# hahnyuan/PTQ4ViT

Measured on AMD Instinct MI355X. Metric: calibration throughput (wrapped modules calibrated per second), ViT-B/224 W8A8, 32 calibration images, higher is better.
Workload: dtype int8

## Files before the change

### include/ptq4vit_hip_debug.h

```cpp
#ifndef PTQ4VIT_HIP_DEBUG_H
#define PTQ4VIT_HIP_DEBUG_H

#include <stddef.h>
#include <stdint.h>

#ifdef __cplusplus
extern "C" {
#endif

int p4v_debug_set_variant(int variant, int force_generic);
int p4v_debug_set_tuning(int key, int value);
int p4v_debug_bound_totals(float* out, int64_t capacity, int64_t* count);
int p4v_debug_set_arena_gap(size_t bytes);
int p4v_debug_arena_ranges(uint64_t* out, int cap);
int p4v_debug_sos_sweep(const p4v_matmul_desc* desc, const float* d_A, const float* d_B, const float* d_out, const float* d_grad,
                        int n_cands, int c_lo, int c_hi, int known_cands, float* d_scores, void* d_workspace, size_t workspace_bytes,
                        void* stream);
int p4v_debug_topk_rows(const float* d_mass, int segs, int n, int k, int32_t* d_idx, void* stream);
int p4v_debug_pack_dual(const float* d_x, long rows, long cols, long cols_padded, int sos, int lo, int hi, int qmax,
                        const float* d_scale, float const_scale, int8_t* d_q1, int8_t* d_q2, void* stream);
int p4v_debug_pack_cands(const float* d_x, long rows, long cols, long rows_padded, long cols_padded, int layout, int lo, int hi,
                         const float* d_scales, int n_cands, const int* d_crange, const unsigned char* d_done, int live_max,
                         int general, int8_t* d_q, void* stream);
int p4v_debug_gather_im2col(int batch, int in_channels, int height, int width, int kernel_h, int kernel_w, int stride_h, int stride_w,
                            int pad_h, int pad_w, int dil_h, int dil_w, const float* d_x, const int32_t* d_idx, int k, float* d_dst,
                            void* stream);
int p4v_debug_prep_epi6(const float* d_o, const float* d_wt, const float* d_bias, long o_ss, long o_ts, int sr, int tr,
                        int bias_on_t, int wt_mode, int transposed, float* d_e, void* stream);

#ifdef __cplusplus
}
#endif
#endif
```

### ptq4vit_amd/_lib.py

```python
import ctypes as C
import os

_HERE = os.path.dirname(os.path.abspath(__file__))
LIB_PATH = os.environ.get("P4V_LIB") or os.path.join(_HERE, "csrc", "libptq4vit_hip.so")

METRICS = {
    "L1_norm": 0,
    "L2_norm": 1,
    "linear_weighted_L2_norm": 2,
    "square_weighted_L2_norm": 3,
    "hessian": 4,
    "cosine": 5,
}


class LinearDesc(C.Structure):
    _fields_ = [(n, C.c_int32) for n in (
        "batch", "tokens", "in_features", "out_features", "n_V", "n_H", "n_a", "w_bit", "a_bit", "metric",
        "eq_n", "search_round", "twin_postgelu", "init_layerwise", "has_bias", "reserved")]


class MatMulDesc(C.Structure):
    _fields_ = ([(n, C.c_int32) for n in ("batch", "heads", "M", "K", "N")] + [("_pad0", C.c_int32)] +
                [("a_stride", C.c_int64 * 4), ("b_stride", C.c_int64 * 4)] +
                [(n, C.c_int32) for n in ("A_bit", "B_bit", "metric", "eq_n", "search_round", "sos",
                                          "init_layerwise", "reserved")])


class MatMulBlocksDesc(C.Structure):
    _fields_ = [("mm", MatMulDesc)] + [(n, C.c_int32) for n in ("n_V_A", "n_H_A", "n_V_B", "n_H_B")]


class ConvDesc(C.Structure):
    _fields_ = [(n, C.c_int32) for n in (
        "batch", "in_channels", "height", "width", "out_channels", "kernel_h", "kernel_w", "stride_h", "stride_w",
        "pad_h", "pad_w", "dil_h", "dil_w", "w_bit", "a_bit", "metric", "eq_n", "search_round", "channelwise",
        "init_layerwise", "has_bias", "reserved")]


class KernelStats(C.Structure):
    _fields_ = [("sweep_i8_ms", C.c_double), ("sweep_i8_launches", C.c_int64), ("sweep_i8_macs", C.c_double),
                ("sweep_f32_ms", C.c_double), ("sweep_f32_launches", C.c_int64), ("sweep_f32_macs", C.c_double),
                ("sweep_i8_alg_macs", C.c_double), ("sweep_f32_alg_macs", C.c_double),
                ("sweep6_ms", C.c_double), ("sweep6_launches", C.c_int64), ("sweep6_macs", C.c_double), ("sweep6_alg_macs", C.c_double),
                ("memo_hits", C.c_int64), ("memo_misses", C.c_int64),
                ("sweep7_ms", C.c_double), ("sweep7_launches", C.c_int64), ("sweep7_macs", C.c_double), ("sweep7_alg_macs", C.c_double),
                ("sweep7_twin_ms", C.c_double), ("sweep7_twin_launches", C.c_int64), ("event_overhead_ms", C.c_double)]


class LaunchRecord(C.Structure):
    _fields_ = [("kind", C.c_int32), ("stage", C.c_int32), ("grid_x", C.c_int32), ("grid_z", C.c_int32),
                ("ms", C.c_double), ("ops", C.c_double), ("alg_ops", C.c_double), ("alg_bytes", C.c_double)]


LAUNCH_KINDS = {0: "k_sweep<int8>", 1: "k_sweep<float>", 2: "k_sweep6", 3: "k_sweep7", 4: "k_sweep7 (twin)", 5: "k_sweep4/5", 6: "k_sweep9",
                7: "k_sweep8", 8: "k_sweep2g", 9: "k_sweep2", 11: "k_sos_split", 12: "k_bound", 13: "k_slice_b", 14: "k_slice_a", 15: "k_sweep_seg"}
LAUNCH_STAGES = {0: "full", 1: "A", 2: "B1", 3: "B2", 4: "A2"}


class PlaneDesc(C.Structure):
    _fields_ = [("rows", C.c_int64), ("cols", C.c_int64), ("cols_padded", C.c_int64), ("rows_per_scale", C.c_int64),
                ("mode", C.c_int32), ("lo", C.c_int32), ("hi", C.c_int32), ("qmax", C.c_int32),
                ("const_scale", C.c_float), ("reserved", C.c_int32)]


class ExportDesc(C.Structure):
    _fields_ = [("dims", C.c_int32 * 4), ("src_stride", C.c_int64 * 4),
                ("scale1_stride", C.c_int64 * 4), ("scale1_div", C.c_int32 * 4),
                ("scale2_stride", C.c_int64 * 4), ("scale2_div", C.c_int32 * 4),
                ("scale2_const", C.c_float),
                ("mode", C.c_int32), ("lo1", C.c_int32), ("hi1", C.c_int32), ("lo2", C.c_int32), ("hi2", C.c_int32),
                ("qmax", C.c_int32), ("reserved", C.c_int32)]


class GroupJob(C.Structure):
    _fields_ = [("kind", C.c_int32), ("status", C.c_int32), ("desc", C.c_void_p), ("inp", C.c_void_p * 5), ("mult", C.c_void_p),
                ("out", C.c_void_p * 3), ("workspace", C.c_void_p), ("workspace_bytes", C.c_size_t)]


JOB_LINEAR, JOB_MATMUL, JOB_CONV, JOB_MATMUL_BLOCKS = 0, 1, 2, 3
PLANE_SYM, PLANE_SOS_HI, PLANE_SOS_LO, PLANE_TWIN = 1, 2, 3, 4
EXPORT_SYM_I8, EXPORT_SYM_F32, EXPORT_GELU_U8, EXPORT_SOS_U8 = 0, 1, 2, 3


EXPORTS = [
    "p4v_version", "p4v_last_error",
    "p4v_linear_workspace_bytes", "p4v_linear_calibrate",
    "p4v_matmul_workspace_bytes", "p4v_matmul_calibrate",
    "p4v_matmul_blocks_workspace_bytes", "p4v_matmul_blocks_calibrate", "p4v_amax_init_matmul_blocks",
    "p4v_matmul_blocks_search", "p4v_matmul_blocks_quant_forward",
    "p4v_conv_workspace_bytes", "p4v_conv_calibrate",
    "p4v_calibrate_group", "p4v_launch_counters",
    "p4v_linear_quant_forward", "p4v_matmul_quant_forward",
    "p4v_amax_init_linear", "p4v_linear_search_w", "p4v_linear_search_a",
    "p4v_amax_init_matmul", "p4v_matmul_search_A", "p4v_sos_search_split", "p4v_matmul_search_B",
    "p4v_amax_init_conv", "p4v_conv_search_w_channelwise", "p4v_conv_search_w_layerwise", "p4v_conv_search_a",
    "p4v_score_argmax_gather",
    "p4v_quantize_i8", "p4v_pack_plane_i8", "p4v_fake_quant", "p4v_export_quantize", "p4v_multi_copy",
    "p4v_stats_enable", "p4v_stats_reset", "p4v_stats_get", "p4v_stats_launches", "p4v_prune_counters",
    "p4v_debug_set_variant", "p4v_debug_set_tuning", "p4v_debug_bound_totals", "p4v_debug_topk_rows", "p4v_debug_pack_dual", "p4v_debug_prep_epi6",
    "p4v_debug_pack_cands", "p4v_debug_gather_im2col", "p4v_debug_sos_sweep",
    "p4v_debug_set_arena_gap", "p4v_debug_arena_ranges",
]

_lib = None


def load():
    global _lib
    if _lib is not None:
        return _lib
    if not os.path.exists(LIB_PATH):
        raise RuntimeError(
            f"ptq4vit_amd: HIP extension {LIB_PATH} is missing -- build it with "
            "`python -c 'import __graft_entry__ as g; g.build()'` (hipcc --offload-arch=gfx950). "
            "There is no CPU fallback for the calibration path.")
    import torch
    lib = C.CDLL(LIB_PATH)
    vp, fp, ip = C.c_void_p, C.c_void_p, C.c_void_p
    lib.p4v_version.restype = C.c_int
    lib.p4v_last_error.restype = C.c_char_p
    lib.p4v_linear_workspace_bytes.restype = C.c_size_t
    lib.p4v_linear_workspace_bytes.argtypes = [C.POINTER(LinearDesc)]
    lib.p4v_linear_calibrate.restype = C.c_int
    lib.p4v_linear_calibrate.argtypes = [C.POINTER(LinearDesc), fp, fp, fp, fp, fp, fp, fp, fp, fp, ip, vp, C.c_size_t, vp]
    lib.p4v_matmul_workspace_bytes.restype = C.c_size_t
    lib.p4v_matmul_workspace_bytes.argtypes = [C.POINTER(MatMulDesc)]
    lib.p4v_matmul_calibrate.restype = C.c_int
    lib.p4v_matmul_calibrate.argtypes = [C.POINTER(MatMulDesc), fp, fp, fp, fp, fp, fp, fp, fp, fp, ip, vp, C.c_size_t, vp]
    MBD = C.POINTER(MatMulBlocksDesc)
    lib.p4v_matmul_blocks_workspace_bytes.restype = C.c_size_t
    lib.p4v_matmul_blocks_workspace_bytes.argtypes = [MBD]
    lib.p4v_matmul_blocks_calibrate.restype = C.c_int
    lib.p4v_matmul_blocks_calibrate.argtypes = [MBD, fp, fp, fp, fp, fp, fp, fp, fp, fp, ip, vp, C.c_size_t, vp]
    lib.p4v_amax_init_matmul_blocks.restype = C.c_int
    lib.p4v_amax_init_matmul_blocks.argtypes = [MBD, fp, fp, fp, fp, vp, C.c_size_t, vp]
    lib.p4v_matmul_blocks_search.restype = C.c_int
    lib.p4v_matmul_blocks_search.argtypes = [MBD, C.c_int32, C.c_int32, C.c_int32] + [fp] * 9 + [ip, vp, C.c_size_t, vp]
    lib.p4v_matmul_blocks_quant_forward.restype = C.c_int
    lib.p4v_matmul_blocks_quant_forward.argtypes = [MBD, fp, fp, fp, fp, fp, fp, vp, C.c_size_t, vp]
    lib.p4v_conv_workspace_bytes.restype = C.c_size_t
    lib.p4v_conv_workspace_bytes.argtypes = [C.POINTER(ConvDesc)]
    lib.p4v_conv_calibrate.restype = C.c_int
    lib.p4v_conv_calibrate.argtypes = [C.POINTER(ConvDesc), fp, fp, fp, fp, fp, fp, fp, fp, fp, ip, vp, C.c_size_t, vp]
    lib.p4v_linear_quant_forward.restype = C.c_int
    lib.p4v_linear_quant_forward.argtypes = [C.POINTER(LinearDesc), fp, fp, fp, fp, fp, fp, vp, C.c_size_t, vp]
    lib.p4v_matmul_quant_forward.restype = C.c_int
    lib.p4v_matmul_quant_forward.argtypes = [C.POINTER(MatMulDesc), fp, fp, fp, fp, fp, fp, vp, C.c_size_t, vp]
    LD, MD, CD = C.POINTER(LinearDesc), C.POINTER(MatMulDesc), C.POINTER(ConvDesc)
    tail = [vp, C.c_size_t, vp]
    for name, args in (
            ("p4v_amax_init_linear", [LD] + [fp] * 4),
            ("p4v_linear_search_w", [LD] + [fp] * 9 + [ip]),
            ("p4v_linear_search_a", [LD] + [fp] * 9 + [ip]),
            ("p4v_amax_init_matmul", [MD] + [fp] * 4),
            ("p4v_matmul_search_A", [MD] + [fp] * 8 + [ip]),
            ("p4v_sos_search_split", [MD] + [fp] * 7 + [ip]),
            ("p4v_matmul_search_B", [MD] + [fp] * 9 + [ip]),
            ("p4v_amax_init_conv", [CD] + [fp] * 4),
            ("p4v_conv_search_w_channelwise", [CD] + [fp] * 9 + [ip]),
            ("p4v_conv_search_w_layerwise", [CD] + [fp] * 9 + [ip]),
            ("p4v_conv_search_a", [CD] + [fp] * 9 + [ip])):
        fn = getattr(lib, name)
        fn.restype = C.c_int
        fn.argtypes = args + tail
    lib.p4v_score_argmax_gather.restype = C.c_int
    lib.p4v_score_argmax_gather.argtypes = [fp, C.c_int32, C.c_int32, fp, fp, ip, vp]
    lib.p4v_quantize_i8.restype = C.c_int
    lib.p4v_quantize_i8.argtypes = [fp, C.c_int64, C.c_int64, C.c_int64, fp, C.c_int64, C.c_int32, C.c_int32, vp, vp]
    lib.p4v_fake_quant.restype = C.c_int
    lib.p4v_fake_quant.argtypes = [fp, C.c_int64, C.c_int64, fp, C.c_int64, C.c_int32, C.c_int32, fp, vp]
    lib.p4v_pack_plane_i8.restype = C.c_int
    lib.p4v_pack_plane_i8.argtypes = [C.POINTER(PlaneDesc), fp, fp, vp, vp]
    lib.p4v_export_quantize.restype = C.c_int
    lib.p4v_export_quantize.argtypes = [C.POINTER(ExportDesc), fp, fp, fp, vp, vp]
    lib.p4v_multi_copy.restype = C.c_int
    lib.p4v_multi_copy.argtypes = [vp, C.c_int32, C.c_int64, C.c_int64, vp]
    lib.p4v_debug_topk_rows.restype = C.c_int
    lib.p4v_debug_topk_rows.argtypes = [vp, C.c_int, C.c_int, C.c_int, vp, vp]
    lib.p4v_debug_pack_dual.restype = C.c_int
    lib.p4v_debug_pack_dual.argtypes = [fp, C.c_long, C.c_long, C.c_long, C.c_int, C.c_int, C.c_int, C.c_int, fp, C.c_float, vp, vp, vp]
    lib.p4v_debug_pack_cands.restype = C.c_int
    lib.p4v_debug_pack_cands.argtypes = [fp, C.c_long, C.c_long, C.c_long, C.c_long, C.c_int, C.c_int, C.c_int, fp, C.c_int, vp, vp,
                                         C.c_int, C.c_int, vp, vp]
    lib.p4v_debug_gather_im2col.restype = C.c_int
    lib.p4v_debug_gather_im2col.argtypes = [C.c_int] * 12 + [fp, ip, C.c_int, fp, vp]
    lib.p4v_debug_sos_sweep.restype = C.c_int
    lib.p4v_debug_sos_sweep.argtypes = [C.POINTER(MatMulDesc), fp, fp, fp, fp, C.c_int, C.c_int, C.c_int, C.c_int, fp, vp, C.c_size_t, vp]
    lib.p4v_debug_prep_epi6.restype = C.c_int
    lib.p4v_debug_prep_epi6.argtypes = [fp, fp, fp, C.c_long, C.c_long, C.c_int, C.c_int, C.c_int, C.c_int, C.c_int, fp, vp]
    lib.p4v_debug_set_variant.restype = C.c_int
    lib.p4v_debug_set_variant.argtypes = [C.c_int, C.c_int]
    lib.p4v_debug_set_tuning.restype = C.c_int
    lib.p4v_debug_set_tuning.argtypes = [C.c_int, C.c_int]
    lib.p4v_debug_set_arena_gap.restype = C.c_int
    lib.p4v_debug_set_arena_gap.argtypes = [C.c_size_t]
    lib.p4v_debug_arena_ranges.restype = C.c_int
    lib.p4v_debug_arena_ranges.argtypes = [C.POINTER(C.c_uint64), C.c_int]
    lib.p4v_debug_bound_totals.restype = C.c_int
    lib.p4v_debug_bound_totals.argtypes = [fp, C.c_int64, C.POINTER(C.c_int64)]
    lib.p4v_stats_enable.restype = C.c_int
    lib.p4v_stats_enable.argtypes = [C.c_int]
    lib.p4v_stats_reset.restype = C.c_int
    lib.p4v_stats_get.restype = C.c_int
    lib.p4v_stats_get.argtypes = [C.POINTER(KernelStats)]
    lib.p4v_stats_launches.restype = C.c_int
    lib.p4v_stats_launches.argtypes = [C.POINTER(LaunchRecord), C.c_int64, C.POINTER(C.c_int64)]
    lib.p4v_prune_counters.restype = C.c_int
    lib.p4v_prune_counters.argtypes = [C.POINTER(C.c_int64), C.c_int]
    lib.p4v_launch_counters.restype = C.c_int
    lib.p4v_launch_counters.argtypes = [C.POINTER(C.c_int64), C.c_int]
    lib.p4v_calibrate_group.restype = C.c_int
    lib.p4v_calibrate_group.argtypes = [C.POINTER(GroupJob), C.c_int32, vp, vp]
    _lib = lib
    return lib


def check(rc, what):
    if rc != 0:
        msg = load().p4v_last_error().decode("utf-8", "replace")
        if rc == -2:
            raise NotImplementedError(f"{what}: {msg}")
        raise RuntimeError(f"{what} failed (code {rc}): {msg}")


def source_hash():
    import hashlib
    root = os.path.dirname(os.path.abspath(__file__))
    h = hashlib.sha256()
    for rel in ("csrc/p4v_kernels.h", "csrc/p4v_api.hip", "../include/ptq4vit_hip.h"):
        with open(os.path.join(root, rel), "rb") as f:
            h.update(f.read())
    return h.hexdigest()[:16]
```

### ptq4vit_amd/csrc/p4v_api.hip

```cpp
#include <hip/hip_runtime.h>

#include <algorithm>
#include <atomic>
#include <climits>
#include <cstdarg>
#include <cstdio>
#include <condition_variable>
#include <cstring>
#include <deque>
#include <functional>
#include <thread>
#include <mutex>
#include <string>
#include <unordered_map>
#include <type_traits>
#include <vector>

#include "../../include/ptq4vit_hip.h"
#include "../../include/ptq4vit_hip_debug.h"
#include "p4v_kernels.h"

using namespace p4v;

namespace {
// ... 4 lines not shown
    char buf[512];
    va_list ap;
    va_start(ap, fmt);
    vsnprintf(buf, sizeof buf, fmt, ap);
    va_end(ap);
    g_err = buf;
    return code;
}

#define HIPCHK(expr)                                                                              \
    do {                                                                                          \
        hipError_t e_ = (expr);                                                                   \
        if (e_ != hipSuccess) return fail(P4V_ERR_HIP, "%s failed: %s", #expr, hipGetErrorString(e_)); \
    } while (0)
#define CHK(expr)              \
    do {                       \
        int r_ = (expr);       \
        if (r_ != 0) return r_; \
    } while (0)

inline long rup(long x, long m) { return (x + m - 1) / m * m; }
inline int cdiv(long a, long b) { return (int)((a + b - 1) / b); }

constexpr size_t WS_ALIGN = 16;
std::atomic<size_t> g_arena_gap{0};
thread_local std::vector<std::pair<size_t, size_t>> g_arena_ranges;
inline void arena_note(size_t b, size_t e) {
    if (e <= b) return;
    auto& v = g_arena_ranges;
    auto it = v.begin();
    while (it != v.end() && it->second < b) ++it;
    if (it == v.end() || it->first > e) { v.insert(it, {b, e}); return; }
    it->first = std::min(it->first, b);
    it->second = std::max(it->second, e);
    auto nx = it + 1;
    while (nx != v.end() && nx->first <= it->second) { it->second = std::max(it->second, nx->second); nx = v.erase(nx); }
}

struct Arena {
    char* base;
    size_t cap, off, peak;
    size_t top;
    bool dry;
    size_t gap;
    Arena(void* b, size_t c) : base((char*)b), cap(c & ~(size_t)255), off(0), peak(0), top(0), dry(b == nullptr),
                               gap(g_arena_gap.load(std::memory_order_relaxed)) {
        if (!dry) g_arena_ranges.clear();
    }
    template <typename T> T* get(size_t n) {
        off = (size_t)rup((long)off, 256);
        T* p = dry ? nullptr : (T*)(base + off);
        if (gap && !dry) arena_note(off, off + n * sizeof(T));
        off += n * sizeof(T) + gap;
        if (off + top > peak) peak = off + top;
        return p;
    }
    char* get_top(size_t bytes) {
        top += (size_t)rup((long)bytes, 256) + gap;
        if (off + top > peak) peak = off + top;
        if (dry || top > cap) return nullptr;
        if (gap) arena_note(cap - top, cap - top + bytes);
        return base + cap - top;
    }
    bool ok() const { return dry || off + top <= cap; }
};

struct StatRec { hipEvent_t a, b; int kind; double macs, alg; int stage, gx, gz; double ms, bytes; };
thread_local double g_alg_bytes = 0;
thread_local double g_alg_macs_cand = 0;
thread_local double g_exec_frac = 1.0;
thread_local bool g_stat_on = false;
thread_local std::vector<StatRec> g_stat_recs;
thread_local std::vector<StatRec> g_stat_done;
thread_local bool g_b1_keep = false;
thread_local std::vector<float> g_b1_totals;
thread_local int g_stage = 0;
thread_local p4v_kernel_stats g_stats = {};
thread_local long g_memo_hits = 0, g_memo_misses = 0;
std::atomic<long long> g_prune_cnt[4];
constexpr int VARIANT_KEPT = 1 | 2 | 4 | 2048 | 32768 | 65536 | 131072 | 524288 | 1048576 | 2097152 | 4194304 | 8388608 | 134217728;
std::atomic<int> g_variant_word{0};
#define g_variant (g_variant_word.load(std::memory_order_relaxed) & 0x3fffffff)
#define g_force_v1 ((g_variant_word.load(std::memory_order_relaxed) >> 30) & 1)
std::atomic<int> g_tune[16];
enum { TUNE_CG6 = 0, TUNE_CG2 = 1, TUNE_CG2G = 2, TUNE_CG7 = 3, TUNE_PRINT = 4, TUNE_ORDER7 = 5, TUNE_P6 = 6, TUNE_PLANE_GIB = 7, TUNE_EPI6W = 8,
       TUNE_LOOSE_PCT = 9, TUNE_SLICE_DIV = 10, TUNE_SLICE_SMALL = 11, TUNE_B1_PATH = 12, TUNE_TIER2 = 13, TUNE_TIER2_DIV = 14, TUNE_LOOSE_ROWS = 15 };
inline bool tune_b1_removed(int v) { return v == 1 || v == 2 || v == 3 || v == 5 || v == 6 || v == 8 || v == 10 || v == 12; }
inline int tune(int k) { return g_tune[k].load(std::memory_order_relaxed); }
inline bool b1_previous() { return tune(TUNE_B1_PATH) == 4; }

inline int ws_aligned(const void* p) {
    return ((uintptr_t)p % WS_ALIGN) == 0 ? 0 : fail(P4V_ERR_INVALID, "d_workspace must be aligned to %zu bytes", WS_ALIGN);
}

struct Group;
struct Ctx {
    hipStream_t st;
    Arena ws;
    bool dry;
    Group* grp = nullptr;
    int slot = 0;
    int par = 1;
};

struct StatInfo { int kind; double macs, alg; int stage, gx, gz; double bytes; };
struct QOp;
struct KernelDesc {
    hipError_t (*one)(const QOp&, hipStream_t);
    hipError_t (*many)(const QOp* const*, int, hipStream_t);
    int cap;
};
constexpr int QOP_PARAM_BYTES = 480;
struct QOp {
    enum Type : int { KERNEL, FILL, D2H, H2D, COPY2D, WAIT };
    int type = KERNEL;
    const KernelDesc* kd = nullptr;
    dim3 grid, block;
    unsigned lds = 0;
    alignas(16) char params[QOP_PARAM_BYTES];
    void* dst = nullptr; const void* src = nullptr; size_t bytes = 0; int value = 0;
    size_t dpitch = 0, spitch = 0, width = 0, height = 0;
    std::vector<char> payload;
    bool timed = false;
    bool heavy = false;
    StatInfo si{};
};
inline hipError_t lds_attr(const void* fn, unsigned lds, std::atomic<bool>& done) {
    if (lds <= 48 * 1024 || done.load(std::memory_order_acquire)) return hipSuccess;
    const hipError_t e = hipFuncSetAttribute(fn, hipFuncAttributeMaxDynamicSharedMemorySize, 160 * 1024);
    if (e == hipSuccess) done.store(true, std::memory_order_release);
    return e;
}
template <typename P, void (*K1)(P), void (*KG)(GroupArgs<P>)> struct Kern {
    static_assert(sizeof(P) <= QOP_PARAM_BYTES, "kernel parameter block larger than a queued operation holds");
    static hipError_t one(const QOp& op, hipStream_t st) {
        static std::atomic<bool> attr{false};
        if (hipError_t e = lds_attr((const void*)K1, op.lds, attr); e != hipSuccess) return e;
        P p;
        std::memcpy(&p, op.params, sizeof(P));
        void* args[] = {&p};
        return hipLaunchKernel((const void*)K1, op.grid, op.block, args, op.lds, st);
    }
    static hipError_t many(const QOp* const* ops, int n, hipStream_t st) {
        static std::atomic<bool> attr{false};
        GroupArgs<P> a;
        unsigned off = 0, lds = 0;
        a.n = n;
        for (int m = 0; m < n; ++m) {
            const QOp& op = *ops[m];
            a.off[m] = off; a.gx[m] = op.grid.x; a.gy[m] = op.grid.y; a.gz[m] = op.grid.z;
            std::memcpy(&a.p[m], op.params, sizeof(P));
            off += (unsigned)rup((long)op.grid.x * op.grid.y * op.grid.z, 8);
            lds = std::max(lds, op.lds);
        }
        a.off[n] = off;
        if (hipError_t e = lds_attr((const void*)KG, lds, attr); e != hipSuccess) return e;
        void* args[] = {&a};
        return hipLaunchKernel((const void*)KG, dim3(off), ops[0]->block, args, lds, st);
    }
    static const KernelDesc* desc() { static const KernelDesc d{&one, &many, GroupArgs<P>::CAP}; return &d; }
};
template <typename P, void (*K1)(P)> struct Kern1 {
    static_assert(sizeof(P) <= QOP_PARAM_BYTES, "kernel parameter block larger than a queued operation holds");
    static hipError_t one(const QOp& op, hipStream_t st) {
        static std::atomic<bool> attr{false};
        if (hipError_t e = lds_attr((const void*)K1, op.lds, attr); e != hipSuccess) return e;
        P p;
        std::memcpy(&p, op.params, sizeof(P));
        void* args[] = {&p};
        return hipLaunchKernel((const void*)K1, op.grid, op.block, args, op.lds, st);
    }
    static const KernelDesc* desc() { static const KernelDesc d{&one, nullptr, 1}; return &d; }
};
#define KERN(P, NAME) (Kern<P, NAME, NAME##_g>::desc())
#define KERN_T(P, NAME, ...) (Kern<P, NAME<__VA_ARGS__>, NAME##_g<__VA_ARGS__>>::desc())
#define KERN1_T(P, NAME, ...) (Kern1<P, NAME<__VA_ARGS__>>::desc())

constexpr int MIR_SLOT = 2048, MIR_SLOTS = 3;
constexpr int MIR_HDR = 160, MIR_BLK = 32, MIR_RB1 = 16, MIR_RB2 = 80;
constexpr size_t MIRROR_BYTES = sizeof(int) * MIR_HDR + sizeof(float) * MIR_SLOT * MIR_SLOTS;
inline int* mirror_alloc() {
    void* p = nullptr;
    if (hipHostMalloc(&p, MIRROR_BYTES, hipHostMallocPortable | hipHostMallocMapped | hipHostMallocCoherent) != hipSuccess) { (void)hipGetLastError(); p = nullptr; }
    return (int*)p;
}

struct Group {
    hipStream_t st = nullptr;
    int n = 0;
    std::mutex mu;
    std::condition_variable cv;
    std::vector<std::deque<QOp>> q;
    std::vector<int> state;
    int blocked = 0;
    unsigned long gen = 0;
    int status = 0;
    std::string err;
    std::vector<int*> mirrors;
    bool stat_on = false;
    std::vector<StatRec>* stat_recs = nullptr;
    long n_ops = 0, n_launches = 0, n_rounds = 0;
    hipEvent_t inputs_ready = nullptr;
    bool waited = false;
    int last_par[16] = {};
    int issue_kernels(std::vector<const QOp*>& ops);
    int issue_round();
    int sync(int slot);
    void finish(int slot);
};

std::atomic<long long> g_launch_cnt[4];
int enqueue_now(hipStream_t st, const QOp& op, bool timed, std::vector<StatRec>* recs) {
    g_launch_cnt[1].fetch_add(1, std::memory_order_relaxed);
    StatRec rec{};
    if (timed) {
        HIPCHK(hipEventCreate(&rec.a));
        HIPCHK(hipEventCreate(&rec.b));
        HIPCHK(hipEventRecord(rec.a, st));
    }
    HIPCHK(op.kd->one(op, st));
    if (timed) {
        HIPCHK(hipEventRecord(rec.b, st));
        rec.kind = op.si.kind; rec.macs = op.si.macs; rec.alg = op.si.alg; rec.stage = op.si.stage; rec.gx = op.si.gx; rec.gz = op.si.gz; rec.bytes = op.si.bytes;
        recs->push_back(rec);
    }
    return 0;
}
int issue_plain(hipStream_t st, const QOp& op) {
    switch (op.type) {
        case QOp::FILL: HIPCHK(hipMemsetAsync(op.dst, op.value, op.bytes, st)); break;
        case QOp::D2H: HIPCHK(hipMemcpyAsync(op.dst, op.src, op.bytes, hipMemcpyDeviceToHost, st)); break;
        case QOp::H2D: HIPCHK(hipMemcpyAsync(op.dst, op.payload.data(), op.bytes, hipMemcpyHostToDevice, st)); break;
        case QOp::COPY2D: HIPCHK(hipMemcpy2DAsync(op.dst, op.dpitch, op.src, op.spitch, op.width, op.height, hipMemcpyDeviceToDevice, st)); break;
        default: break;
    }
    return 0;
}
int Group::issue_kernels(std::vector<const QOp*>& ops) {
    const KernelDesc* kd = ops[0]->kd;
    const int total = (int)ops.size();
    if (ops[0]->heavy && ops[0]->si.kind >= 0 && ops[0]->si.kind < 16) last_par[ops[0]->si.kind] = total;
    if (!kd->many || total == 1) {
        for (const QOp* op : ops) { CHK(enqueue_now(st, *op, op->timed && stat_recs, stat_recs)); ++n_launches; }
        return 0;
    }
    const int chunks = cdiv(total, kd->cap), per = cdiv(total, chunks);
    for (int i0 = 0; i0 < total; i0 += per) {
        const int m = std::min(per, total - i0);
        bool timed = stat_recs != nullptr;
        for (int i = 0; i < m; ++i) timed = timed && ops[i0 + i]->timed;
        StatRec rec{};
        if (timed) {
            HIPCHK(hipEventCreate(&rec.a));
            HIPCHK(hipEventCreate(&rec.b));
            HIPCHK(hipEventRecord(rec.a, st));
        }
        HIPCHK(kd->many(ops.data() + i0, m, st));
        g_launch_cnt[1].fetch_add(1, std::memory_order_relaxed);
        ++n_launches;
        if (timed) {
            HIPCHK(hipEventRecord(rec.b, st));
            const StatInfo& s0 = ops[i0]->si;
            rec.kind = s0.kind; rec.stage = s0.stage; rec.gz = m;
            for (int i = 0; i < m; ++i) {
                const QOp& o = *ops[i0 + i];
                rec.macs += o.si.macs; rec.alg += o.si.alg; rec.bytes += o.si.bytes;
                rec.gx += (int)rup((long)o.grid.x * o.grid.y * o.grid.z, 8);
            }
            stat_recs->push_back(rec);
        }
    }
    return 0;
}
int Group::issue_round() {
    ++n_rounds;
    g_launch_cnt[2].fetch_add(1, std::memory_order_relaxed);
    std::vector<const QOp*> bucket;
    for (;;) {
        int best = -1, best_n = 0;
        bool best_heavy = true;
        int n_wait = 0, n_live = 0;
        for (int i = 0; i < n; ++i) {
            if (q[i].empty()) continue;
            ++n_live;
            const QOp& h = q[i].front();
            if (h.type == QOp::WAIT) { ++n_wait; continue; }
            if (h.type != QOp::KERNEL) { best = i; best_n = 0; break; }
            if (h.heavy && !best_heavy) continue;
            int cnt = 0;
            for (int j = i; j < n; ++j)
                if (!q[j].empty()) { const QOp& o = q[j].front(); cnt += o.type == QOp::KERNEL && o.kd == h.kd && o.block.x == h.block.x && o.block.y == h.block.y && o.block.z == h.block.z; }
            if ((best_heavy && !h.heavy) || cnt > best_n) { best = i; best_n = cnt; best_heavy = h.heavy; }
        }
        if (best < 0 && n_wait > 0) {
            if (!waited && inputs_ready) { HIPCHK(hipStreamWaitEvent(st, inputs_ready, 0)); waited = true; }
            for (int i = 0; i < n; ++i)
                if (!q[i].empty() && q[i].front().type == QOp::WAIT) q[i].pop_front();
            continue;
        }
        if (best < 0) break;
        const QOp& h = q[best].front();
        if (h.type != QOp::KERNEL) {
            const int r = issue_plain(st, h);
            ++n_ops;
            q[best].pop_front();
            if (r) return r;
            continue;
        }
        bucket.clear();
        std::vector<int> who;
        for (int j = best; j < n; ++j)
            if (!q[j].empty()) { const QOp& o = q[j].front(); if (o.type == QOp::KERNEL && o.kd == h.kd && o.block.x == h.block.x && o.block.y == h.block.y && o.block.z == h.block.z) { bucket.push_back(&o); who.push_back(j); } }
        n_ops += (long)bucket.size();
        const int r = issue_kernels(bucket);
        for (int j : who) q[j].pop_front();
        if (r) return r;
    }
    return 0;
}
int Group::sync(int slot) {
    std::unique_lock<std::mutex> lk(mu);
    state[slot] = 1;
    ++blocked;
    if (blocked == n) {
// ... 114 lines not shown
        case P4V_METRIC_LINEAR_WEIGHTED_L2: *epi = EPI_W_SQ; *wt_mode = 3; break;
        case P4V_METRIC_SQUARE_WEIGHTED_L2: *epi = EPI_SQ_W; *wt_mode = 2; break;
        case P4V_METRIC_HESSIAN: *epi = EPI_SQ_W; *wt_mode = 1; break;
        default: *epi = EPI_COS; *wt_mode = 0; break;
    }
}

int launch_absmax(Ctx& c, const float* src, const long (&st)[4], int D0, int D1, int R, int C, int nV, int nH,
                  int crb_r, int crb_c, int signed_max, unsigned* out) {
    if (c.dry) return 0;
    CHK(q_fill(c, out, 0, sizeof(unsigned) * (size_t)D1 * nV * nH));
    AbsMaxParams p{src, st[0], st[1], st[2], st[3], D0, D1, R, C, nV, nH, crb_r, crb_c, 0, signed_max, out};
    p.row_tile = std::max(1, std::min(crb_r, std::max(1, 8192 / std::max(1, std::min(crb_c, C)))));
    const int tiles_per_v = cdiv(crb_r, p.row_tile);
    dim3 grid(tiles_per_v * nV * nH, D1, D0);
    return enqueue(c, KERN(AbsMaxParams, k_absmax), grid, dim3(256), 0, p);
}

int launch_interval(Ctx& c, const unsigned* enc, int n, float denom, int broadcast, float* interval) {
    if (c.dry) return 0;
    return enqueue(c, KERN(IntervalParams, k_interval_from_max), dim3(cdiv(n, 64)), dim3(64), 0, IntervalParams{enc, n, denom, broadcast, interval});
}

int launch_cands(Ctx& c, const float* mult, const float* interval, int ncand, int nblk, float* cands) {
    if (c.dry) return 0;
    return enqueue(c, KERN(CandsParams, k_make_cands), dim3(cdiv((long)ncand * nblk, 256)), dim3(256), 0, CandsParams{mult, interval, ncand, nblk, cands});
}

int launch_scale(Ctx& c, ScaleParams p) {
    if (c.dry) return 0;
    return enqueue(c, KERN(ScaleParams, k_scale_table), dim3(cdiv((long)p.C * p.nblk, 256)), dim3(256), 0, p);
}

std::atomic<int> g_cvt_state{0};
void cvt_probe(hipStream_t stream) {
    if (g_cvt_state.load(std::memory_order_acquire) != 0) return;
    static std::mutex mu;
    std::lock_guard<std::mutex> lk(mu);
    if (g_cvt_state.load(std::memory_order_acquire) != 0) return;
    static unsigned* scratch = nullptr;
    if (!scratch && hipMalloc(&scratch, 8 * sizeof(unsigned)) != hipSuccess) { (void)hipGetLastError(); scratch = nullptr; return; }
    unsigned h[5] = {9, 9, 9, 9, 9};
    hipLaunchKernelGGL(k_probe_cvt, dim3(1), dim3(64), 0, stream, scratch);
    if (hipGetLastError() != hipSuccess || hipMemcpyAsync(h, scratch, sizeof h, hipMemcpyDeviceToHost, stream) != hipSuccess ||
        hipStreamSynchronize(stream) != hipSuccess) { (void)hipGetLastError(); return; }
    const bool sat = h[3] == 0 && h[4] == 255;
    const int st = (sat && h[0] == 0 && h[1] == 1 && h[2] == 2) ? 1 : (sat && h[0] == 1 && h[1] == 2 && (h[2] == 2 || h[2] == 3)) ? 2 : 3;
    if (tune(TUNE_PRINT) > 0) fprintf(stderr, "[p4v] v_cvt_pk_u8_f32(0.7, 1.5, 2.5, -3, 300) = %u %u %u %u %u -> mode %d\n", h[0], h[1], h[2], h[3], h[4], st);
    g_cvt_state.store(st, std::memory_order_release);
}
float cvt_bias(Ctx& c) {
    if (!c.dry && !c.grp) cvt_probe(c.st);
    const int st = g_cvt_state.load(std::memory_order_acquire);
    return st == 1 ? 128.5f : st == 2 ? 128.0f : 0.0f;
}
inline bool pack1_ok(const PackParams& p, int live_max) {
    return p.mode == PACK_SYM && !p.conv && !(p.blk_mode == 1 && p.blk_div2) && p.lo >= -128 && p.hi <= 127 && p.lo <= p.hi &&
           (p.crange ? live_max == 1 : p.C == 1) && (p.c_inner != 3 || (p.Rp % 64 == 0 && p.Kp % 64 == 0));
}
std::atomic<int> g_pack_general{0};
template <typename T> int launch_pack(Ctx& c, const PackParams& p_, int live_max = -1) {
    if (c.dry) return 0;
    PackParams p = p_;
    if (p.crange && live_max == 0) return 0;
    p.qbias = (sizeof(T) == 1 && p.mode == PACK_SYM && p.lo == -128 && p.hi == 127 && tune(TUNE_B1_PATH) != 11) ? cvt_bias(c) : 0.0f;
    const long total = (long)p.Z * p.Rp * (p.Kp / 16);
    if (total >= (1L << 31)) return fail(P4V_ERR_UNSUPPORTED, "operand plane too large for k_pack (%ld 16-element runs)", total);
    const int groups = cdiv((p.crange && live_max > 0) ? std::min(p.C, live_max) : p.C, PACK_CG);
    const long cap = !p.crange ? 256L * 64 : live_max > 0 ? std::max(256L * 12, 256L * 64 / groups) : 256L * 12;
    const int blocks = (int)std::min<long>(cdiv(total, 256), cap);
    if (p.mode == PACK_TWIN_I8) {
        if (sizeof(T) != 1 || p.C != 1 || p.c_inner != 0 || !p.scales || p.conv || p.zdiv > 0)
            return fail(P4V_ERR_UNSUPPORTED, "merged twin plane: one fixed row-major int8 plane only");
        return enqueue(c, KERN(PackParams, k_pack_twin), dim3(blocks), dim3(256), 0, p);
    }
    const bool single = sizeof(T) == 1 && pack1_ok(p, live_max) && !g_pack_general.load(std::memory_order_relaxed);
    if (tune(TUNE_PRINT) > 1) fprintf(stderr, "[p4v] %s stage %d: Z %d Rp %d Kp %d C %d crange %d done %d live_max %d layout %d grid %d x %d\n", single ? "k_pack1" : "k_pack", g_stage, p.Z, p.Rp, p.Kp, p.C, p.crange != nullptr, p.done != nullptr, live_max, p.c_inner, blocks, single ? 1 : groups);
    if (single) return enqueue(c, KERN(PackParams, k_pack1), dim3(blocks), dim3(256), 0, p);
    return enqueue(c, KERN_T(PackParams, k_pack, T), dim3(blocks, groups), dim3(256), 0, p);
}

inline int lockstep(const Ctx& c, int kind) {
    if (!c.grp) return 1;
    const int seen = (kind >= 0 && kind < 16) ? c.grp->last_par[kind] : 0;
    return std::max(1, seen > 0 ? seen : c.par);
}
inline int cu_slots(const Ctx& c, int slots, int kind) { return std::max(8, slots / lockstep(c, kind)); }
#define P4V_EPI4(epi, X)                                   \
    switch (epi) {                                         \
        case EPI_SQ_W: { constexpr int E = EPI_SQ_W; X; }  \
        case EPI_SQ: { constexpr int E = EPI_SQ; X; }      \
        case EPI_ABS: { constexpr int E = EPI_ABS; X; }    \
        default: { constexpr int E = EPI_W_SQ; X; }        \
    }

template <typename T, bool TWIN> int launch_sweep_epi(Ctx& c, const SweepParams& p, int epi, int cgroups, const StatInfo* si) {
    const size_t lds = 2 * (TWIN ? 3 : 2) * SW_TILE_BYTES;
    dim3 grid(p.mtiles * p.ntiles, p.Z, cgroups), block(512);
    switch (epi) {
        case EPI_SQ_W: return enqueue(c, KERN_T(SweepParams, k_sweep, T, TWIN, EPI_SQ_W), grid, block, lds, p, si);
        case EPI_SQ: return enqueue(c, KERN_T(SweepParams, k_sweep, T, TWIN, EPI_SQ), grid, block, lds, p, si);
        case EPI_ABS: return enqueue(c, KERN_T(SweepParams, k_sweep, T, TWIN, EPI_ABS), grid, block, lds, p, si);
        case EPI_W_SQ: return enqueue(c, KERN_T(SweepParams, k_sweep, T, TWIN, EPI_W_SQ), grid, block, lds, p, si);
        case EPI_STORE: return enqueue(c, KERN1_T(SweepParams, k_sweep, T, TWIN, EPI_STORE), grid, block, lds, p, si);
        case EPI_FWD: return enqueue(c, KERN1_T(SweepParams, k_sweep, T, TWIN, EPI_FWD), grid, block, lds, p, si);
        default: return enqueue(c, KERN1_T(SweepParams, k_sweep, T, TWIN, EPI_COS), grid, block, lds, p, si);
    }
}

template <bool TWIN> int launch_sweep2g_epi(Ctx& c, const SweepParams& p, int epi, int cgroups, const StatInfo* si) {
    const int per = 2 * cdiv(p.c1 - p.c0, 2 * cgroups);
    const size_t lds = (size_t)SW2_NS * (TWIN ? 4 : 3) * SW2_TILE + (size_t)per * 8 * sizeof(float) * (TWIN ? 3 : 2);
    dim3 grid(p.mtiles * p.ntiles, p.Z, cgroups), block(512);
    P4V_EPI4(epi, return enqueue(c, KERN_T(SweepParams, k_sweep2g, TWIN, E), grid, block, lds, p, si))
}

template <bool TWIN> int launch_sweep2_epi(Ctx& c, const SweepParams& p, int epi, int cgroups, const StatInfo* si) {
    const int per = cdiv(p.c1 - p.c0, cgroups);
    const size_t lds = (size_t)SW2_NS * (TWIN ? 3 : 2) * SW2_TILE + (size_t)per * 8 * sizeof(float) * (TWIN ? 3 : 2);
    dim3 grid(p.mtiles * p.ntiles, p.Z, cgroups), block(512);
    switch (epi) {
        case EPI_SQ_W: return enqueue(c, KERN_T(SweepParams, k_sweep2, TWIN, EPI_SQ_W), grid, block, lds, p, si);
        case EPI_SQ: return enqueue(c, KERN_T(SweepParams, k_sweep2, TWIN, EPI_SQ), grid, block, lds, p, si);
        case EPI_ABS: return enqueue(c, KERN_T(SweepParams, k_sweep2, TWIN, EPI_ABS), grid, block, lds, p, si);
        case EPI_FWD: return enqueue(c, KERN1_T(SweepParams, k_sweep2, TWIN, EPI_FWD), grid, block, lds, p, si);
        case EPI_STORE:
            if constexpr (TWIN) return enqueue(c, KERN1_T(SweepParams, k_sweep2, TWIN, EPI_STORE), grid, block, lds, p, si);
            else return enqueue(c, KERN_T(SweepParams, k_sweep2, TWIN, EPI_STORE), grid, block, lds, p, si);
        case EPI_COS: return enqueue(c, KERN_T(SweepParams, k_sweep2, TWIN, EPI_COS), grid, block, lds, p, si);
        default: return enqueue(c, KERN_T(SweepParams, k_sweep2, TWIN, EPI_W_SQ), grid, block, lds, p, si);
    }
}

#ifdef P4V_TRACE
unsigned long long* g_trace = nullptr;
int trace_attach(Sweep3Params& p) {
    if (!g_trace) HIPCHK(hipMalloc(&g_trace, sizeof(unsigned long long) * 16 * 65536));
    p.trace = g_trace;
    return 0;
}
int trace_dump(Ctx& c, dim3 grid, int ktiles) {
    if (!getenv("P4V_TRACE_FILE")) return 0;
    const size_t n = (size_t)grid.x * grid.z * 16;
    HIPCHK(hipStreamSynchronize(c.st));
    std::vector<unsigned long long> h(n);
    HIPCHK(hipMemcpy(h.data(), g_trace, n * 8, hipMemcpyDeviceToHost));
    FILE* f = fopen(getenv("P4V_TRACE_FILE"), "ab");
    unsigned long long hdr[4] = {0xABCDull, grid.x, grid.z, (unsigned long long)ktiles};
    fwrite(hdr, 8, 4, f); fwrite(h.data(), 8, n, f); fclose(f);
    return 0;
}
#endif

inline StatInfo stat_info(int kind, double macs, double alg, int gx, int gz, double bytes) {
    return StatInfo{kind, macs * g_exec_frac, alg * g_exec_frac, g_stage, gx, gz, bytes};
}

enum SweepKind { SK_BOUND, SK_SWEEP6, SK_SWEEP5, SK_SWEEP7, SK_SWEEP7_TWIN, SK_SWEEP7_MERGED, SK_SWEEP9, SK_SWEEP8, SK_SWEEP2G, SK_SWEEP2,
                 SK_GENERIC_I8, SK_GENERIC_F32, SK_COUNT };
constexpr int SWEEP_RECORD_KIND[SK_COUNT] = {12, 2, 5, 3, 4, 4, 6, 7, 8, 9, 0, 1};
inline bool sweep_stationary(SweepKind k) { return k == SK_SWEEP6 || k == SK_SWEEP5; }
inline bool sweep_large_k(SweepKind k) { return k == SK_SWEEP7 || k == SK_SWEEP7_TWIN || k == SK_SWEEP7_MERGED; }

int launch_sweep5(Ctx& c, const Sweep3Params& p, int epi, int cgroups) {
    if (c.dry) return 0;
    const int per = 2 * cdiv(p.c1 - p.c0, 2 * cgroups);
    const size_t lds = (size_t)p.ktiles * SW2_TILE + (size_t)SW5_NP * 2 * SW2_TILE + (size_t)per * 8 * sizeof(float) * 2 + 256;
// ... 176 lines not shown
}

struct PlaneCache {
    char* buf = nullptr;
    bool assigned = false, valid = false;
    unsigned char* done = nullptr;
};
struct SliceCache {
    bool assigned = false;
    int k = 0;
    int k_eff = 0;
    int* idx = nullptr; float* mass = nullptr; float* mass_u = nullptr;
    float* Os = nullptr; float* Gs = nullptr; float* Rs = nullptr; float* Cs = nullptr;
    const void* idx_src = nullptr; int idx_wt = -1;
    const void* o_src = nullptr; const void* g_src = nullptr; const void* r_src = nullptr; const void* c_src = nullptr;
    float* frac = nullptr;
    PlaneCache aplane;
    bool loose = false;
    float frac_host = 1.0f;
};
typedef PlaneCache EpiCache;

struct Operand {
    PackParams pk;
    bool expanded;
    bool present;
};

struct SegPlan {
    SegTable seg; unsigned char ablk[SEG_MAX], bblk[SEG_MAX]; int Kseg;
    int batch, H, M, K, N;
    int nVA, nHA, nVB, nHB, crA, ccA, crB, ccB;
    const float* A; long a_st[4]; const float* B; long b_st[4];
    int Aq, Bq; bool sos;
    const float* ivA; const float* ivB;
    const float* split;
    int side, ov_v, ov_h;
    const float* cands; int cand_cs, cand_hs;
    bool b_shared;
};

struct Pass {
    bool i8, twin;
    int epi, wt_mode;
    Operand row, row2, col;
    int Z;
    long row_zs_shared, col_zs_shared;
    int Mrows, Ncols, K;
    int eq_n;
    ScaleParams s1, s2;
    bool use_s1;
    int sb_mode, sb_div, s_cs;
    const float* bias; int bias_axis; long bias_zs;
    const float* O; const float* G;
    long o_zs, o_bs, o_ms, o_nbs, o_ns; int o_inner, o_ninner;
    int j_mode, j_div, nj; double norm;
    int cos_ZB, cos_ZV, cos_j_mode, cos_j_div;
    const float* cands; int cand_cs, cand_js, cand_off;
    float* interval; int out_js, out_off;
    float* aux_out; float aux_div;
    float* scores_out; int scores_out_ld;
    int32_t* best_out;
    float* store_out;
    bool cos6;
    bool cos7;
    bool twin_disjoint;
    const int* crange;
    const int* crange_blk;
    int host_lo, host_hi;
    const int* host_rblk;
    int host_len;
    float* scores_keep;
    bool no_select;
    bool prunable;
    bool prunable_f32;
    float* S1_pre; float* S2_pre; bool s_ready;
    SliceCache* scache;
    SliceCache* scache2;
    bool bound_kernel;
    bool host_sync_ok;
    PlaneCache* cache;
    EpiCache* ecache;
    bool pack_only;
    const SegPlan* seg;
};

static const long PLANE_BUDGET_DEFAULT = 6L << 30;
#define PLANE_BUDGET (tune(TUNE_PLANE_GIB) > 0 ? ((long)tune(TUNE_PLANE_GIB) << 30) : PLANE_BUDGET_DEFAULT)
#define PLANE_CACHE_MAX (PLANE_BUDGET / 2)

int choose_cgroups(long wgs, int ncand, int ktiles, int slots, double prologue_us, double tile_us, int cg_max = 25) {
    int best = 1;
    double best_t = 1e30;
    for (int cg = 1; cg <= std::min(ncand, cg_max); ++cg) {
        const long rounds = (wgs * cg + slots - 1) / slots;
        const double t = (double)rounds * (prologue_us + (double)cdiv(ncand, cg) * ktiles * tile_us);
        if (t < best_t * 0.999) { best_t = t; best = cg; }
    }
    return best;
}

bool dual_pack_ok(const PackParams& a, const PackParams& b) {
    auto plain = [](const PackParams& p) {
        return (p.mode == PACK_SYM || p.mode == PACK_SOS_HI || p.mode == PACK_SOS_LO) && p.blk_mode == 0 && !p.conv && !p.crange;
    };
    return plain(a) && plain(b) && a.src == b.src && a.R == b.R && a.K == b.K && a.s_r == b.s_r && a.s_k == b.s_k &&
           a.s_z == b.s_z && a.s_z2 == b.s_z2 && a.zdiv == b.zdiv;
}

int launch_pass_select(Ctx& c, const Pass& ps, const float* scores) {
    SelectParams sl{scores, ps.eq_n, ps.nj, ps.cands, ps.cand_cs, ps.cand_js, ps.cand_off, ps.interval, ps.out_js,
                    ps.out_off, ps.aux_out, ps.aux_div, ps.scores_out, ps.scores_out_ld, ps.best_out};
    return launch_select(c, sl);
}

int launch_pack_seg(Ctx& c, PackSegParams p) {
    if (c.dry) return 0;
    p.qbias = (p.mode == PACK_SYM && p.lo == -128 && p.hi == 127) ? cvt_bias(c) : 0.0f;
    const long total = (long)p.Z * p.Rp * (p.Kseg / 16);
    if (total >= (1L << 31)) return fail(P4V_ERR_UNSUPPORTED, "operand plane too large for k_pack_seg (%ld 16-element runs)", total);
    const int groups = cdiv(p.C, PACK_CG);
    return enqueue(c, KERN(PackSegParams, k_pack_seg), dim3((unsigned)std::min<long>(cdiv(total, 256), 256L * 64), groups), dim3(256), 0, p);
}
template <bool TWIN> int launch_sweep_seg_epi(Ctx& c, const SweepSegParams& p, int epi, int cgroups, const StatInfo* si) {
    const size_t lds = 2 * (TWIN ? 3 : 2) * SW_TILE_BYTES + 2 * SEG_MAX * 128 * sizeof(float) + SEG_KT_MAX * sizeof(short) + 2 * SEG_MAX;
    dim3 grid(p.mtiles * p.ntiles, p.Z, cgroups), block(512);
    if (epi == EPI_FWD) return enqueue(c, KERN_T(SweepSegParams, k_sweep_seg, TWIN, EPI_FWD), grid, block, lds, p, si);
    if constexpr (!TWIN) { if (epi == EPI_COS) return enqueue(c, KERN_T(SweepSegParams, k_sweep_seg, false, EPI_COS), grid, block, lds, p, si); }
    if (epi == EPI_COS) return fail(P4V_ERR_UNSUPPORTED, "k_sweep_seg: the cosine epilogue has no twin instance");
    P4V_EPI4(epi, return enqueue(c, KERN_T(SweepSegParams, k_sweep_seg, TWIN, E), grid, block, lds, p, si))
}
int run_pass_seg(Ctx& c, Pass& ps) {
    const SegPlan& g = *ps.seg;
    const int Z = ps.Z, M = g.M, N = g.N, H = g.H, Kseg = g.Kseg;
    const bool fwd = ps.epi == EPI_FWD, cosm = ps.epi == EPI_COS;
    const int ZB = g.b_shared ? 1 : Z;
    g_alg_macs_cand = (double)M * N * g.K * Z;
    g_alg_bytes = 4.0 * ((double)M * g.K * Z + (double)N * g.K * ZB) + (ps.G ? 8.0 : 4.0) * (double)M * N * Z;
    const int Mp = (int)rup(M, SW_BM), Np = (int)rup(N, SW_BN), MT = cosm ? cdiv(M, 64) : Mp / 64;
    const long a_plane = (long)Z * Mp * Kseg, b_plane = (long)ZB * Np * Kseg;
    const bool a_exp = g.side == 1, b_exp = g.side == 2;
    const long exp_plane = a_exp ? a_plane : b_plane;
    const int chunk = (int)std::max<long>(1, std::min<long>(ps.eq_n, PLANE_BUDGET / std::max<long>(1, exp_plane)));
    const size_t mark = c.ws.off;
    char* abuf = c.ws.get<char>((size_t)a_plane * (a_exp ? chunk : 1));
    char* a2buf = g.sos ? c.ws.get<char>((size_t)a_plane) : nullptr;
    char* bbuf = c.ws.get<char>((size_t)b_plane * (b_exp ? chunk : 1));
    const long p_zs = (long)MT * Np * (cosm ? 3 : 1), p_cs = p_zs * Z;
    float* part = fwd ? nullptr : c.ws.get<float>((size_t)p_cs * ps.eq_n);
    float* scores = fwd ? nullptr : c.ws.get<float>((size_t)ps.eq_n * H);
    if (!c.ws.ok()) return fail(P4V_ERR_WORKSPACE, "workspace too small: need >= %zu bytes", c.ws.off);
    if (c.dry) { c.ws.off = mark; return 0; }

    auto a_pack = [&](int mode, char* dst, const float* cands, int C) {
        PackSegParams p{};
        p.src = g.A; p.s_z2 = g.a_st[0]; p.s_z = g.a_st[1]; p.s_r = g.a_st[2]; p.s_k = g.a_st[3]; p.zdiv = H;
        p.Z = Z; p.R = M; p.K = g.K; p.Rp = Mp; p.Kseg = Kseg; p.dst = dst; p.C = C;
        p.H = H; p.mode = mode; p.seg = g.seg;
        std::memcpy(p.kblk, g.ablk, sizeof p.kblk);
        if (mode == PACK_SYM) {
            p.iv = g.ivA; p.iv_hs = g.nVA * g.nHA; p.iv_rs = g.nHA; p.iv_ks = 1; p.r_div = g.crA; p.nblk_r = g.nVA;
            p.cands = cands; p.cand_cs = g.cand_cs; p.cand_hs = g.cand_hs; p.ov_r = g.ov_v; p.ov_k = g.ov_h;
            p.lo = -g.Aq; p.hi = g.Aq - 1;
        } else {
            p.iv = g.split; p.iv_hs = p.iv_rs = p.iv_ks = 0; p.r_div = std::max(1, M); p.nblk_r = 1;
            p.qm1 = (float)(g.Aq - 1);
// ... 391 lines not shown
    return launch_sweep7(c, q, pl.kind == SK_SWEEP7_MERGED ? 2 : ps.twin ? 1 : 0, ps.epi, cg7);
}

int sweep_chunk_tiled(Ctx& c, const Pass& ps, const SweepPlan& pl, const PassBufs& b, SweepKind kind, int c0, int nc) {
    const int esz = pl.esz, Mp = pl.Mp, Np = pl.Np, Kp = pl.Kp;
    SweepParams sp{};
    sp.a_cs = ps.row.expanded ? pl.row_plane1 : 0;
    sp.A = b.row - (long)c0 * sp.a_cs;
    sp.a_zs = ps.row_zs_shared ? 0 : (long)Mp * Kp * esz;
    if (ps.twin) {
        sp.a2_cs = ps.row2.expanded ? pl.row_plane1 : 0;
        sp.A2 = b.row2 - (long)c0 * sp.a2_cs;
        sp.a2_zs = sp.a_zs;
    }
    sp.b_cs = ps.col.expanded ? pl.col_plane1 : 0;
    sp.B = b.col - (long)c0 * sp.b_cs;
    sp.b_zs = ps.col_zs_shared ? 0 : (long)pl.NpB * Kp * esz;
    sp.b_rows = pl.b64 ? 64 : 0;
    sp.ldk = Kp * esz; sp.ktiles = sp.ldk / SW_BKB;
    sp.S1 = b.S1; sp.S2 = b.S2; sp.s_cs = ps.s_cs; sp.sb_mode = ps.sb_mode; sp.sb_div = std::max(1, ps.sb_div);
    sp.bias = ps.bias; sp.bias_axis = ps.bias_axis; sp.bias_zs = ps.bias_zs;
    sp.O = ps.O; sp.Wt = ps.G ? ps.G : ps.O; sp.wt_mode = ps.wt_mode;
    sp.o_zs = ps.o_zs; sp.o_bs = ps.o_bs; sp.o_ms = ps.o_ms; sp.o_nbs = ps.o_nbs; sp.o_ns = ps.o_ns;
    sp.o_inner = ps.o_inner > 0 ? ps.o_inner : INT_MAX;
    sp.o_ninner = ps.o_ninner > 0 ? ps.o_ninner : INT_MAX;
    sp.M = ps.Mrows; sp.N = ps.Ncols; sp.Z = ps.Z; sp.c0 = c0; sp.c1 = c0 + nc; sp.crange = ps.crange;
    sp.crange_blk = pl.rblk_z; sp.cb_div = std::max(1, ps.j_div);
    sp.part = b.part; sp.p_cs = pl.p_cs; sp.p_zs = pl.p_zs; sp.Np = pl.NpP;
    sp.mtiles = Mp / SW_BM; sp.ntiles = Np / SW_BN;
    sp.dbg = g_variant & 3;
    sp.store = ps.store_out;
    const long wgs = (long)sp.mtiles * sp.ntiles * ps.Z;
    int cgroups;
    switch (kind) {
        case SK_GENERIC_I8: case SK_GENERIC_F32:
            cgroups = choose_cgroups(wgs, nc, sp.ktiles, cu_slots(c, 512, SWEEP_RECORD_KIND[kind]), 20.0, ps.i8 ? 1.6 : 2.6);
            break;
        case SK_SWEEP9:
            sp.halves = pl.h9;
            sp.rows_p_stream = sp.a_cs == 0 ? Np : Mp;
            cgroups = choose_cgroups((long)pl.h9 * ps.Z, nc, 1, cu_slots(c, SW9_NW == 4 ? 512 : 256, SWEEP_RECORD_KIND[SK_SWEEP9]), 12.0, 0.9);
            break;
        case SK_BOUND:
            sp.bound = 1;
            sp.dbg = tune(TUNE_B1_PATH) >= 16 ? (tune(TUNE_B1_PATH) >> 4) : 0;
            sp.A = b.row; sp.B = b.col; sp.a_cs = sp.b_cs = 0;
            [[fallthrough]];
        default:
            cgroups = choose_cgroups(wgs, nc, sp.ktiles, cu_slots(c, ps.twin ? 256 : 512, SWEEP_RECORD_KIND[SK_SWEEP2]), ps.twin ? 40.0 : 25.0, ps.twin ? 0.45 : 0.40);
    }
    const bool tuned = kind != SK_GENERIC_I8 && kind != SK_GENERIC_F32 && !pl.fast_cos && !ps.store_out;
    if (tuned) {
        const char* g = kind == SK_SWEEP2G ? "g" : "";
        if (const int t_ = tune(kind == SK_SWEEP2G ? TUNE_CG2G : TUNE_CG2); t_ > 0) cgroups = std::max(1, std::min(nc, t_));
        if (tune(TUNE_PRINT) > 0) fprintf(stderr, "[p4v] sweep2%s tiles %d x %d z %d ktiles %d cand %d twin %d -> cgroups %d\n", g, sp.mtiles, sp.ntiles, ps.Z, sp.ktiles, nc, (int)ps.twin, cgroups);
    }
    return launch_sweep(c, sp, kind, ps.twin, ps.epi, cgroups);
}

int finish_pass(Ctx& c, const Pass& ps, const SweepPlan& pl, const PassBufs& b) {
    if (ps.epi == EPI_COS) {
        FinishCosParams fp{b.part, pl.p_cs, pl.fin_zs, pl.fin_ld, pl.fin_rows, ps.cos_ZB, ps.cos_ZV, pl.fin_cols, ps.eq_n,
                           ps.cos_j_mode, pl.fin_jdiv, ps.nj, ps.norm, b.scores};
        return launch_finish_cos(c, fp);
    }
    FinishParams fp{b.part, pl.p_cs, pl.fin_zs, pl.fin_ld, pl.fin_rows, ps.Z, pl.fin_cols, ps.eq_n, ps.j_mode, pl.fin_jdiv, ps.nj, ps.norm,
                    b.scores, ps.crange};
    if (ps.crange && b.pc && b.pc->done) { fp.mark_done = b.pc->done; fp.mark_n = ps.eq_n; }
    fp.crange_blk = pl.rblk ? pl.rblk : pl.rblk_z;
    return launch_finish(c, fp);
}

int run_pass(Ctx& c, Pass& ps) {
    if (ps.seg) return run_pass_seg(c, ps);
    g_alg_macs_cand = (double)ps.Mrows * ps.Ncols * ps.K * ps.Z;
    g_alg_bytes = 4.0 * ((double)ps.Mrows * ps.K * (ps.row_zs_shared ? 1 : ps.Z) + (double)ps.Ncols * ps.K * (ps.col_zs_shared ? 1 : ps.Z)) +
                  (ps.G ? 8.0 : 4.0) * (double)ps.Mrows * ps.Ncols * ps.Z;
    SweepPlan pl;
    CHK(plan_sweep(c, ps, pl));
    const size_t mark = c.ws.off;
    PassBufs b{};
    CHK(pass_workspace(c, ps, pl, b));
    if (ps.pack_only) {
        if (b.pc && ps.row.expanded != ps.col.expanded && !ps.crange) CHK(pack_expanded(c, ps, pl, b, 0, ps.eq_n));
        c.ws.off = mark;
        return 0;
    }
    CHK(prep_epilogue(c, ps, pl, b));
    if (ps.use_s1 && !ps.s_ready) {
        ps.s1.S = b.S1; ps.s1.C = ps.eq_n; ps.s1.nblk = ps.s_cs;
        CHK(launch_scale(c, ps.s1));
        if (ps.twin) { ps.s2.S = b.S2; ps.s2.C = ps.eq_n; ps.s2.nblk = ps.s_cs; CHK(launch_scale(c, ps.s2)); }
    }
    CHK(pack_fixed_planes(c, ps, pl, b));
    for (int c0 = 0; c0 < ps.eq_n; c0 += pl.chunk) {
        const int nc = std::min(pl.chunk, ps.eq_n - c0);
        CHK(pack_expanded(c, ps, pl, b, c0, nc));
        CHK(chunk_exec_frac(c, ps, pl, c0, nc));
        const SweepKind kind = chunk_kind(pl, nc);
        if (sweep_stationary(kind)) CHK(sweep_chunk_stationary(c, ps, pl, b, c0, nc));
        else if (sweep_large_k(kind)) CHK(sweep_chunk_large_k(c, ps, pl, b, c0, nc));
        else CHK(sweep_chunk_tiled(c, ps, pl, b, kind, c0, nc));
    }
    g_exec_frac = 1.0;
    if (!ps.store_out) {
        CHK(finish_pass(c, ps, pl, b));
        if (!ps.no_select) CHK(launch_pass_select(c, ps, b.scores));
    }
    c.ws.off = mark;
    return 0;
}

struct SliceGeo {
    bool lin; int segs, seg_rows, k , Ncols, K;
    const float* O; const float* G; int wt_mode; long o_ms;
    const float* row_src; long s_r, s_k; int zdiv; long s_z2, s_z;
    bool conv; PackParams conv_pk;
    int k_cap;
};
int slice_alloc(Ctx& c, SliceCache* sc, const SliceGeo& g, bool keep, bool bump) {
    if (sc->assigned) {
        if (sc->k != g.k_cap) return fail(P4V_ERR_INVALID, "slice cache reused with another geometry");
        return 0;
    }
    if (!keep && !bump) return 0;
    const long zrows = (long)g.segs * g.seg_rows, out_elems = (long)g.segs * g.k_cap * g.Ncols, row_elems = (long)g.segs * g.k_cap * g.K;
    if (keep) {
        sc->idx = reinterpret_cast<int*>(c.ws.get_top((size_t)g.segs * g.k_cap * sizeof(int)));
        sc->mass = reinterpret_cast<float*>(c.ws.get_top((size_t)zrows * sizeof(float)));
        sc->Os = reinterpret_cast<float*>(c.ws.get_top((size_t)out_elems * sizeof(float)));
        sc->Gs = reinterpret_cast<float*>(c.ws.get_top((size_t)out_elems * sizeof(float)));
        sc->Rs = reinterpret_cast<float*>(c.ws.get_top((size_t)row_elems * sizeof(float)));
        sc->frac = reinterpret_cast<float*>(c.ws.get_top(256));
        sc->assigned = true;
    } else {
        sc->idx = c.ws.get<int>((size_t)g.segs * g.k_cap);
        sc->mass = c.ws.get<float>((size_t)zrows);
        sc->Os = c.ws.get<float>((size_t)out_elems);
        sc->Gs = c.ws.get<float>((size_t)out_elems);
        sc->Rs = c.ws.get<float>((size_t)row_elems);
    }
    sc->k = g.k_cap;
    return 0;
}
int slice_fill(Ctx& c, SliceCache* sc, const SliceGeo& g, bool host_sync_ok) {
    const long zrows = (long)g.segs * g.seg_rows;
    const void* wsrc = g.G ? (const void*)g.G : (const void*)g.O;
    const bool new_idx = sc->idx_src != wsrc || sc->idx_wt != g.wt_mode || (g.wt_mode != 1 && sc->o_src != g.O);
    if (new_idx) {
        CHK(enqueue(c, KERN(RowMassParams, k_row_mass), dim3((unsigned)cdiv(zrows, 4)), dim3(256), 0, RowMassParams{g.G ? g.G : g.O, g.O, zrows, (long)g.Ncols, g.wt_mode, sc->mass}));
        CHK(enqueue(c, KERN(TopkParams, k_topk_rows), dim3(g.segs), dim3(1024), 0, TopkParams{sc->mass, g.seg_rows, g.k, sc->idx}));
        sc->idx_src = wsrc; sc->idx_wt = g.wt_mode;
        sc->o_src = sc->g_src = sc->r_src = nullptr;
        if (sc->frac && host_sync_ok && !(g_variant & 8388608)) {
            float f = 1.0f;
            int* hm = host_mirror(c);
            CHK(enqueue(c, KERN(MassFracParams, k_mass_fraction), dim3(1), dim3(1024), 0,
                        MassFracParams{sc->mass, zrows, sc->idx, g.segs, g.seg_rows, g.k, sc->frac, hm ? reinterpret_cast<float*>(hm + 4) : nullptr}));
            if (!hm) CHK(q_d2h(c, &f, sc->frac, sizeof f));
            CHK(q_sync(c));
            if (hm) f = *reinterpret_cast<volatile float*>(hm + 4);
            if (tune(TUNE_PRINT) > 0) fprintf(stderr, "[p4v] slice holds %.4f of the metric weight (%d x %d of %d rows)\n", f, g.segs, g.k, g.seg_rows);
            sc->frac_host = f;
            if (g.k < g.k_cap && !(f >= 0.97f)) {
                SliceGeo g2 = g;
                g2.k = g.k_cap;
                sc->idx_src = nullptr;
// ... 79 lines not shown
        pk.Rp = 16; pk.Kp = Kp; pk.dst = dst; pk.Z = Z; pk.C = 1; pk.c_inner = 0;
        return launch_pack<int8_t>(c, pk);
    };
    CHK(pack16(a.row, A1));
    if (a.twin) CHK(pack16(a.row2, A2));
    if (!c.dry) {
        const PackParams& b = a.col.pk;
        SliceBParams kp{};
        kp.A = A1; kp.A2 = A2;
        kp.B = b.src; kp.b_z2 = b.s_z2; kp.b_z = b.s_z; kp.b_n = b.s_r; kp.b_k = b.s_k; kp.zdiv = b.zdiv;
        kp.bscale = b.scales; kp.bs_cs = b.sc_cs; kp.bs_div = b.blk_div; kp.lo = b.lo; kp.hi = b.hi;
        kp.S1 = S1; kp.S2 = S2; kp.s_cs = a.s_cs; kp.s_div = a.sb_div;
        kp.O = a.O; kp.Wt = a.G ? a.G : a.O; kp.wt_mode = a.wt_mode;
        kp.Z = Z; kp.M = a.Mrows; kp.K = a.K; kp.Kp = Kp; kp.N = a.Ncols; kp.C = a.eq_n; kp.part = part;
        const int nb = cdiv(a.Ncols, 16);
        const int slots = std::max(8, 256 * (a.twin ? 2 : 3) / lockstep(c, 13));
        int groups = std::max(1, std::min(a.eq_n / 10, cdiv(std::max(1, 512 / lockstep(c, 13)), Z)));
        while ((long)Z * groups < 4L * slots && groups < a.eq_n / 10 && ((long)Z * groups) % slots != 0 && ((long)Z * groups) % slots < slots * 3 / 4) ++groups;
        if (tune(TUNE_CG2) > 0) groups = std::max(1, std::min(a.eq_n, tune(TUNE_CG2)));
        const dim3 grid(Z, groups), block(256);
        const float qbias = (b.lo == -128 && b.hi == 127 && tune(TUNE_B1_PATH) != 11) ? cvt_bias(c) : 0.0f;
        const StatInfo si{13, 16.0 * nb * 16 * Kp * Z * a.eq_n * (a.twin ? 2 : 1), (double)a.Mrows * a.Ncols * a.K * Z * a.eq_n, g_stage, Z, groups,
                          4.0 * ((double)a.Mrows * a.K * Z + (double)a.Ncols * a.K * Z) + (a.G ? 8.0 : 4.0) * (double)a.Mrows * a.Ncols * Z};
        const StatInfo* sp = &si;
        int r_ = 0;
        SliceB2Params kp2{kp, qbias};
#define P4V_LAUNCH_SB2(TW, KTM, NBW)                                                                                                  \
        P4V_EPI4(a.epi, r_ = (qbias != 0.0f) ? enqueue(c, KERN_T(SliceB2Params, k_slice_b2, TW, KTM, NBW, E, true), grid, block, 0, kp2, sp)   \
                                             : enqueue(c, KERN_T(SliceB2Params, k_slice_b2, TW, KTM, NBW, E, false), grid, block, 0, kp2, sp); break)
        if (Kp == 64) { if (a.twin) { P4V_LAUNCH_SB2(true, 1, 4) } else { P4V_LAUNCH_SB2(false, 1, 4) } }
        else { if (a.twin) { P4V_LAUNCH_SB2(true, 4, 1) } else { P4V_LAUNCH_SB2(false, 4, 1) } }
#undef P4V_LAUNCH_SB2
        if (r_) return r_;
    }
    FinishParams fp{part, (long)Z * 4, 4L, 4, 1, Z, 4, a.eq_n, a.j_mode, std::max(1, a.j_div), a.nj, a.norm, SA, nullptr};
    CHK(launch_finish(c, fp));
    c.ws.off = mark;
    return 0;
}

bool slice_a_ok(const Pass& a) {
    const PackParams& r = a.row.pk;
    return a.i8 && a.row.expanded && !a.col.expanded && !a.twin && a.Z > 1 && a.Mrows <= 16 && !a.store_out &&
           a.epi != EPI_COS && a.epi != EPI_STORE && a.epi != EPI_FWD && !a.bias && a.use_s1 && a.sb_mode == 2 && a.j_mode == 2 &&
           a.sb_div == a.j_div && a.s_cs == a.sb_div && !a.crange && a.scores_keep && a.no_select &&
           !r.conv && r.mode == PACK_SYM && r.blk_mode == 2 && r.blk_div == a.sb_div && r.scales && r.s_k == 1 && r.s_r == a.K &&
           r.zdiv > 0 && r.s_z == (long)a.Mrows * a.K && r.s_z2 == (long)r.zdiv * a.Mrows * a.K && a.Mrows == 16 &&
           !a.col_zs_shared && !a.row_zs_shared && a.K <= 64 && a.Ncols <= 208 && a.o_ms == a.Ncols && a.o_ns == 1 &&
           a.o_zs == (long)a.Mrows * a.Ncols && !a.o_bs && !a.o_nbs && !g_force_v1;
}
int run_slice_a(Ctx& c, Pass& a, float* SA) {
    const int Z = a.Z, nb = cdiv(a.Ncols, 16);
    const size_t mark = c.ws.off;
    int8_t* Bp = c.ws.get<int8_t>((size_t)Z * nb * 16 * 64);
    float* part = c.ws.get<float>((size_t)a.eq_n * Z);
    float* S1 = a.S1_pre ? a.S1_pre : c.ws.get<float>((size_t)a.eq_n * a.s_cs);
    if (!c.ws.ok()) return fail(P4V_ERR_WORKSPACE, "workspace too small: need >= %zu bytes", c.ws.off);
    if (!a.s_ready) {
        a.s1.S = S1; a.s1.C = a.eq_n; a.s1.nblk = a.s_cs;
        CHK(launch_scale(c, a.s1));
    }
    {
        PackParams pk = a.col.pk;
        pk.Rp = nb * 16; pk.Kp = 64; pk.dst = Bp; pk.Z = Z; pk.C = 1; pk.c_inner = 0;
        CHK(launch_pack<int8_t>(c, pk));
    }
    if (!c.dry) {
        const PackParams& r = a.row.pk;
        SliceAParams kp{};
        kp.A = r.src; kp.B = Bp;
        kp.ascale = r.scales; kp.as_cs = r.sc_cs; kp.as_div = r.blk_div; kp.lo = r.lo; kp.hi = r.hi;
        kp.S1 = S1; kp.s_cs = a.s_cs; kp.s_div = a.sb_div;
        kp.O = a.O; kp.Wt = a.G ? a.G : a.O; kp.wt_mode = a.wt_mode;
        kp.Z = Z; kp.M = a.Mrows; kp.K = a.K; kp.N = a.Ncols; kp.C = a.eq_n; kp.part = part;
        kp.qbias = (r.lo == -128 && r.hi == 127 && tune(TUNE_B1_PATH) != 11) ? cvt_bias(c) : 0.0f;
        const int groups = std::max(1, std::min(a.eq_n / 4, cdiv(std::max(1, 1024 / lockstep(c, 14)), Z)));
        const dim3 grid(Z, groups), block(256);
        const StatInfo si{14, 16.0 * nb * 16 * 64 * Z * a.eq_n, (double)a.Mrows * a.Ncols * a.K * Z * a.eq_n, g_stage, Z, groups,
                          4.0 * ((double)a.Mrows * a.K * Z + (double)a.Ncols * a.K * Z) + (a.G ? 8.0 : 4.0) * (double)a.Mrows * a.Ncols * Z};
        const StatInfo* sp = &si;
        P4V_EPI4(a.epi, CHK(enqueue(c, KERN_T(SliceAParams, k_slice_a, 13, E), grid, block, 0, kp, sp)); break)
    }
    FinishParams fp{part, (long)Z, 1L, 1, 1, Z, 1, a.eq_n, a.j_mode, std::max(1, a.j_div), a.nj, a.norm, SA, nullptr};
    CHK(launch_finish(c, fp));
    c.ws.off = mark;
    return 0;
}

int run_pass_pruned_impl(Ctx& c, Pass& ps);
int run_pass_pruned(Ctx& c, Pass& ps) {
    if (!(g_variant & 134217728) || !prune_ok(ps) || (!c.dry && !ps.interval)) return run_pass_pruned_impl(c, ps);
    const int n = ps.out_off + (std::max(1, ps.nj) - 1) * ps.out_js + 1;
    std::vector<float> keep;
    CHK(run_pass_pruned_impl(c, ps));
    if (!c.dry) CHK(prune_crosscheck_begin(c, ps.interval, n, keep));
    Pass full = ps;
    full.prunable = false; full.scache = nullptr; full.scache2 = nullptr; full.cache = nullptr; full.ecache = nullptr;
    CHK(run_pass(c, full));
    return c.dry ? 0 : prune_crosscheck_end(c, ps.interval, n, keep, "search pass");
}
int run_pass_pruned_impl(Ctx& c, Pass& ps) {
    if (!prune_ok(ps)) { PRUNE_COUNT(3); return run_pass(c, ps); }
    const bool lin = ps.Z == 1;
    const int segs = lin ? 1 : ps.Z;
    const int seg_rows = ps.Mrows;
    int k;
    if (lin) {
        k = (int)std::min<long>(rup(std::max(1, ps.Mrows / (tune(TUNE_SLICE_DIV) > 0 ? tune(TUNE_SLICE_DIV) : 16)), 256), rup(ps.Mrows, 256));
        if ((long)k * 5 > (long)ps.Mrows * 2) { PRUNE_COUNT(2); return run_pass(c, ps); }
        const bool conv_rows = ps.row.pk.conv && ps.row.pk.Z == 1 && !ps.twin;
        if (ps.o_ms != ps.Ncols || ps.o_ns != 1 || ps.o_bs || ps.o_nbs || ps.row.pk.zdiv > 0 ||
            (!conv_rows && (ps.row.pk.conv || ps.row.pk.s_k != 1 || ps.row.pk.s_r != ps.K))) { PRUNE_COUNT(2); return run_pass(c, ps); }
    } else {
        k = 16;
        if (ps.Mrows < 64 || ps.row_zs_shared || ps.o_zs != (long)ps.Mrows * ps.Ncols || ps.o_ms != ps.Ncols || ps.o_ns != 1 ||
            ps.o_bs || ps.o_nbs || ps.row.pk.zdiv <= 0 || ps.row.pk.conv) { PRUNE_COUNT(2); return run_pass(c, ps); }
    }
    SliceCache local;
    SliceCache* sc = ps.scache ? ps.scache : &local;
    if (sc->loose) { PRUNE_COUNT(2); return run_pass(c, ps); }
    const int k_cap = k;
    if (sc->k_eff > 0) k = sc->k_eff;
    else if (lin && ps.scache && ps.host_sync_ok && !c.dry && k_cap >= 512 && !(g_variant & 8388608))
        k = tune(TUNE_SLICE_SMALL) > 0 ? std::min(tune(TUNE_SLICE_SMALL), k_cap)
                                       : (int)std::min<long>(std::max<long>(128, rup(ps.Mrows / 64, 64)), k_cap / 2);
    SliceGeo geo{lin, segs, seg_rows, k, ps.Ncols, ps.K, ps.O, ps.G, ps.wt_mode, ps.o_ms, ps.row.pk.src, ps.row.pk.s_r, ps.row.pk.s_k,
                 ps.row.pk.zdiv, ps.row.pk.s_z2, ps.row.pk.s_z, lin && ps.row.pk.conv != 0, ps.row.pk, k_cap};
    CHK(slice_alloc(c, sc, geo, ps.scache != nullptr, false));
    SliceCache* sc2 = (lin && ps.scache && ps.scache2 && !ps.row.pk.conv && tune(TUNE_TIER2) != 1) ? ps.scache2 : nullptr;
    const int k2 = (int)rup(std::max(1, ps.Mrows / (tune(TUNE_TIER2_DIV) > 0 ? tune(TUNE_TIER2_DIV) : 4)), 256);
    if (sc2 && (k2 < 2 * k_cap || (long)k2 * 5 > (long)ps.Mrows * 2)) sc2 = nullptr;
    SliceGeo geo2 = geo;
    geo2.k = geo2.k_cap = k2;
    if (sc2) CHK(slice_alloc(c, sc2, geo2, true, false));
    const size_t mark = c.ws.off;
    const size_t tab = (size_t)ps.eq_n * std::max(1, ps.nj);
    float* SA = c.ws.get<float>(tab);
    float* SB = c.ws.get<float>(tab);
    float* S2 = c.ws.get<float>(tab);
    float* SA2 = sc2 ? c.ws.get<float>(tab) : nullptr;
    int* r1 = c.ws.get<int>(6);
    int* r2 = r1 + 2;
    int* r3 = r1 + 4;
    int* best_idx = c.ws.get<int>((size_t)std::max(1, ps.nj));
    int* rblk2 = c.ws.get<int>((size_t)4 * std::max(1, ps.nj));
    int* rblk3 = rblk2 + 2 * std::max(1, ps.nj);
    float* vrow = c.ws.get<float>((size_t)std::max(1, ps.cand_cs));
    float* S1s = ps.use_s1 ? c.ws.get<float>((size_t)ps.eq_n * ps.s_cs) : nullptr;
    float* S2s = (ps.use_s1 && ps.twin) ? c.ws.get<float>((size_t)ps.eq_n * ps.s_cs) : nullptr;
    if (!ps.scache) CHK(slice_alloc(c, sc, geo, false, true));
    if (!c.ws.ok()) return fail(P4V_ERR_WORKSPACE, "workspace too small: need >= %zu bytes", c.ws.off);
    float *Os = sc->Os, *Gs = ps.G ? sc->Gs : nullptr, *Rs = sc->Rs;
    Pass a = ps;
    if (!c.dry) {
        CHK(slice_fill(c, sc, geo, ps.host_sync_ok));
        if (sc->loose) { c.ws.off = mark; PRUNE_COUNT(2); return run_pass(c, ps); }
        if (sc->k_eff > 0) k = sc->k_eff;
    }
    PRUNE_COUNT(0);
    a.O = Os; a.G = ps.G ? Gs : nullptr;
    a.Mrows = k;
    auto sliced = [&](PackParams& pk) {
        pk.src = Rs; pk.R = k; pk.s_k = 1; pk.s_r = ps.K; pk.conv = 0;
        if (!lin) { pk.s_z = (long)k * ps.K; pk.s_z2 = (long)pk.zdiv * k * ps.K; }
    };
    sliced(a.row.pk);
    if (ps.twin) sliced(a.row2.pk);
    if (!lin) a.o_zs = (long)k * ps.Ncols;
    a.cache = ps.col.expanded ? ps.cache : (ps.cache && ps.scache) ? &sc->aplane : nullptr;
    a.ecache = nullptr; a.scores_keep = SA; a.no_select = true;
    a.S1_pre = S1s; a.S2_pre = S2s; a.s_ready = false;
    const bool virt = ps.nj > 1 && ps.cand_off == 0 && ps.cand_js * ps.nj == ps.cand_cs && ps.cand_cs <= 4096;
    PruneParams pp{SA, SB, ps.eq_n, ps.nj, prune_margin(), r1, r1, virt ? 1 : 0, best_idx, ps.cands, ps.cand_cs, ps.cand_js, ps.cand_off, vrow};
    g_stage = 1;
    { const int r_ = slice_b_ok(a) ? run_slice_b(c, a, SA) : slice_a_ok(a) ? run_slice_a(c, a, SA) : run_pass(c, a); g_stage = 0; if (r_) return r_; }
    CHK(enqueue(c, KERN(PruneParams, k_prune_pick), dim3(1), dim3(256), 0, pp));
    Pass b1 = ps;
    b1.scores_keep = SB; b1.no_select = true;
    if (!virt) { b1.S1_pre = S1s; b1.S2_pre = S2s; b1.s_ready = true; }
    if (virt) {
        b1.eq_n = 1; b1.cache = nullptr;
        auto swap = [&](const float*& ptr) { if (ptr == ps.cands) ptr = vrow; };
        swap(b1.row.pk.scales); swap(b1.row2.pk.scales); swap(b1.col.pk.scales);
        swap(b1.s1.x); swap(b1.s1.y); swap(b1.s2.x); swap(b1.s2.y);
        b1.cands = vrow;
    } else { b1.crange = r1; if (ps.nj == 1) b1.host_len = 1; }
    if (lin && ps.i8 && !ps.twin && (virt || ps.nj == 1)) { b1.bound_kernel = true; b1.cache = nullptr; b1.ecache = nullptr; }
    g_stage = 2;
    { const int r_ = run_pass(c, b1); g_stage = 0; if (r_) return r_; }
    if (g_b1_keep && !c.dry && !c.grp) {
        std::vector<float> h((size_t)b1.eq_n * std::max(1, ps.nj));
        CHK(q_d2h(c, h.data(), SB, sizeof(float) * h.size()));
        CHK(q_sync(c));
        for (float v : h) if (v != -INFINITY) g_b1_totals.push_back(v);
    }
    pp.r_out = r2; pp.rblk = rblk2;
    int* hm = (ps.host_sync_ok && !c.dry) ? host_mirror(c) : nullptr;
    pp.r_host = hm; pp.rblk_host = hm ? hm + MIR_RB1 : nullptr;
    int hblk[2 * MIR_BLK] = {};
    int hlo = 0, hhi = 0;
    bool hblk_ok = false;
    const bool hull_selects = !ps.scores_out && ps.interval && (virt || ps.nj <= 32);
    SelectParams hsl{SB, ps.eq_n, ps.nj, ps.cands, ps.cand_cs, ps.cand_js, ps.cand_off, hull_selects ? ps.interval : nullptr,
                     ps.out_js, ps.out_off, ps.aux_out, ps.aux_div, nullptr, 0, ps.best_out};
    attach_mirror(hsl);
    CHK(enqueue(c, KERN(HullParams, k_prune_hull), dim3(1), dim3(256), 0, HullParams{pp, hsl}));
    auto select_without_b2 = [&]() -> int {
        PRUNE_COUNT(1);
        if (hull_selects) {}
        else if (virt) {
            CHK(enqueue(c, KERN(FillParams, k_fill_f32), dim3(cdiv((long)tab, 256)), dim3(256), 0, FillParams{S2, -INFINITY, (int)tab}));
            CHK(enqueue(c, KERN(MergeVirtParams, k_merge_virtual), dim3(cdiv(ps.nj, 64)), dim3(64), 0, MergeVirtParams{S2, SB, best_idx, ps.nj}));
            CHK(launch_pass_select(c, ps, S2));
        } else CHK(launch_pass_select(c, ps, SB));
        c.ws.off = mark;
        return 0;
    };
    int nsurv = 0;
    if (ps.host_sync_ok && !c.dry) {
        int h[2] = {0, 1};
        if (!hm) CHK(q_d2h(c, h, r2, sizeof h));
        CHK(q_sync(c));
        if (hm) { h[0] = reinterpret_cast<volatile int*>(hm)[0]; h[1] = reinterpret_cast<volatile int*>(hm)[1]; }
        if (h[0] >= h[1]) return select_without_b2();
        nsurv = h[1] - h[0];
        hlo = h[0]; hhi = h[1];
        if (hm && ps.nj <= MIR_BLK) { for (int i = 0; i < 2 * ps.nj; ++i) hblk[i] = reinterpret_cast<volatile int*>(hm)[MIR_RB1 + i]; hblk_ok = true; }
    }
    const int* rB = r2;
    const int* rBblk = rblk2;
    const int t2min = tune(TUNE_TIER2) >= 2 ? tune(TUNE_TIER2) : 8;
    if (sc2 && (c.dry || (ps.host_sync_ok && nsurv >= t2min && sc->frac_host < 0.9f))) {
        if (!c.dry) CHK(slice_fill(c, sc2, geo2, false));
        Pass a2 = ps;
        a2.O = sc2->Os; a2.G = ps.G ? sc2->Gs : nullptr; a2.Mrows = k2;
        auto sliced2 = [&](PackParams& pk) { pk.src = sc2->Rs; pk.R = k2; pk.s_k = 1; pk.s_r = ps.K; pk.conv = 0; };
        sliced2(a2.row.pk);
        if (ps.twin) sliced2(a2.row2.pk);
        a2.cache = ps.col.expanded ? ps.cache : ps.cache ? &sc2->aplane : nullptr;
        a2.ecache = nullptr; a2.scores_keep = SA2; a2.no_select = true; a2.crange = r2; a2.crange_blk = rblk2;
        int hblk_a2[2 * MIR_BLK];
        std::copy(hblk, hblk + 2 * MIR_BLK, hblk_a2);
        a2.host_lo = hlo; a2.host_hi = hhi; a2.host_rblk = hblk_ok ? hblk_a2 : nullptr;
        a2.S1_pre = S1s; a2.S2_pre = S2s; a2.s_ready = true;
        g_stage = 4;
        { const int r_ = run_pass(c, a2); g_stage = 0; if (r_) return r_; }
        if (!c.dry) {
            PruneParams pp2 = pp;
            pp2.SA = SA2; pp2.r_out = r3; pp2.r_host = hm ? hm + 2 : nullptr; pp2.rblk = rblk3; pp2.rblk_host = hm ? hm + MIR_RB2 : nullptr;
            CHK(enqueue(c, KERN(HullParams, k_prune_hull), dim3(1), dim3(256), 0, HullParams{pp2, hsl}));
            int h[2] = {0, 1};
            if (!hm) CHK(q_d2h(c, h, r3, sizeof h));
            CHK(q_sync(c));
            if (hm) { h[0] = reinterpret_cast<volatile int*>(hm)[2]; h[1] = reinterpret_cast<volatile int*>(hm)[3]; }
            if (tune(TUNE_PRINT) > 0) fprintf(stderr, "[p4v] second tier: %d survivors of the %d-row slice -> %d of the %d-row slice (M %d N %d K %d)\n", nsurv, k, std::max(0, h[1] - h[0]), k2, ps.Mrows, ps.Ncols, ps.K);
            if (h[0] >= h[1]) return select_without_b2();
            rB = r3; rBblk = rblk3;
            hlo = h[0]; hhi = h[1];
// ... 349 lines not shown
    float* Ufold = nullptr;
    float *w_mix = nullptr, *a_mix = nullptr;
    float* Ot = nullptr;
    SegPlan sgp{};
    SearchRounds rounds;
    PlaneCache plane[2];
    EpiCache ecache[2];
    SliceCache slice, slice2;

    LinearCall(Ctx& c_, const p4v_linear_desc* d_, const Stage& sg_) : c(c_), d(d_), sg(sg_) {}

    int build(const float* W_, const float* bias_, const float* X_, const float* O_, const float* G_, const float* mult_, float* w_iv_,
              float* a_iv_, float* scores_out, int32_t* best_out, float* fwd_out_) {
        W = W_; bias = bias_; X = X_; O = O_; G = G_; mult = mult_; w_iv = w_iv_; a_iv = a_iv_; fwd_out = fwd_out_;
        M = d->batch * d->tokens; K = d->in_features; N = d->out_features;
        nV = d->n_V; nH = d->n_H; nA = d->n_a;
        if (M <= 0 || K <= 0 || N <= 0 || nV <= 0 || nH <= 0 || nA <= 0 || d->eq_n <= 0)
            return fail(P4V_ERR_INVALID, "linear: non-positive dimension");
        if (N % nV || K % nH || K % nA) return fail(P4V_ERR_UNSUPPORTED, "linear: n_V/n_H/n_a must divide the layer (reference ignores remainders, linear.py:118)");
        if (d->w_bit > 8 || d->a_bit > 8 || d->w_bit < 2 || d->a_bit < 2) return fail(P4V_ERR_UNSUPPORTED, "linear: bit widths 2..8 supported");
        crb_rows = N / nV; crb_cols = K / nH; crb_acts = K / nA;
        wq = 1 << (d->w_bit - 1); aq = 1 << (d->a_bit - 1);
        a_neg = (float)(0.16997124254703522 / aq);
        metric_epi(d->metric, &epi, &wt_mode);
        cosm = epi == EPI_COS;
        if (wt_mode == 1 && !G && !fwd_out && sg.searches()) return fail(P4V_ERR_INVALID, "linear: hessian metric needs raw_grad (linear.py:418)");
        general = (nH > 1 || nA > 1 || (d->reserved & 1) || (cosm && d->twin_postgelu && !fwd_out));
        i8 = !general;
        twin = d->twin_postgelu && i8;
        segcos = cosm && !fwd_out && (nH > 1 || nA > 1);
        if (segcos && d->twin_postgelu)
            return fail(P4V_ERR_UNSUPPORTED, "linear: cosine with n_H>1 / n_a>1 on the post-GELU twin is not implemented on the GPU "
                                             "(the twin's second plane lies on the column side, k_sweep_seg has no instance for that)");
        if (segcos) {
            if (nH > 8 || nA > 8) return fail(P4V_ERR_UNSUPPORTED, "linear: cosine with up to n_H, n_a = 8 blocks is implemented on the GPU");
            sgp.batch = 1; sgp.H = nV; sgp.M = crb_rows; sgp.K = K; sgp.N = M;
            sgp.nVA = 1; sgp.nHA = nH; sgp.nVB = nA; sgp.nHB = 1;
            sgp.crA = crb_rows; sgp.ccA = crb_cols; sgp.crB = crb_acts; sgp.ccB = M;
            sgp.A = W; sgp.a_st[0] = 0; sgp.a_st[1] = (long)crb_rows * K; sgp.a_st[2] = K; sgp.a_st[3] = 1;
            sgp.B = X; sgp.b_st[0] = 0; sgp.b_st[1] = 0; sgp.b_st[2] = 1; sgp.b_st[3] = K; sgp.b_shared = true;
            sgp.Aq = wq; sgp.Bq = aq; sgp.ivA = w_iv; sgp.ivB = a_iv;
            CHK(seg_cut_k(sgp, "linear"));
        }
        rounds = SearchRounds(sg, d->search_round, d->reserved, d->eq_n, nV, c, scores_out, best_out);
        only_blk = sg.full() ? -1 : ((d->reserved >> 8) & 15) - 1;
        if (sg.searches() && only_blk >= ((sg.mask & ST_S1) ? nH : nA)) return fail(P4V_ERR_INVALID, "linear: block %d outside the layer's blocks", only_blk);
        tab_blk = std::max(0, only_blk);
        cos6 = cosm && i8 && !twin && !general && nH == 1 && nA == 1 && (nV == 1 || crb_rows % 64 == 0) &&
               sweep6_supported((int)(rup(K, 64) / 64)) && !(g_variant & (4 | 2048)) && !g_force_v1;
        cos7 = cosm && i8 && !twin && !general && nH == 1 && nA == 1 && (nV == 1 || crb_rows % 128 == 0) && !cos6 &&
               rup(K, 64) >= 1024 && rup(K, 64) % 256 == 0 && N % 32 == 0 && (long)M * N * 4 < (1L << 32) &&
               (c.dry || (((unsigned long long)O) & 15) == 0) && !(g_variant & (2048 | 32768)) && !g_force_v1;
        ncand = d->eq_n + 1;
        cvt_bias(c);
        enc_w = c.ws.get<unsigned>((size_t)nV * nH);
        enc_a = c.ws.get<unsigned>((size_t)nA);
        w_cands_ws = c.ws.get<float>((size_t)ncand * nV * nH);
        a_cands_ws = c.ws.get<float>((size_t)ncand * nA);
        w_cands = (sg.mask & ST_INIT) ? w_cands_ws : sg.cands1;
        a_cands = (sg.mask & ST_INIT) ? a_cands_ws : sg.cands2;
        Ufold = twin ? c.ws.get<float>((size_t)M * N) : nullptr;
        w_mix = c.ws.get<float>((size_t)ncand * nV * nH);
        a_mix = c.ws.get<float>((size_t)ncand * nA);
        Ot = segcos ? c.ws.get<float>((size_t)M * N) : nullptr;
        if (!c.ws.ok()) return fail(P4V_ERR_WORKSPACE, "workspace too small");
        return 0;
    }

    int init_side(int side) {
        if (fwd_out || !(sg.mask & ST_INIT)) return 0;
        const long stw[4] = {0, 0, K, 1};
        if (side == 0) {
            CHK(launch_absmax(c, W, stw, 1, 1, N, K, nV, nH, crb_rows, crb_cols, 0, enc_w));
            CHK(launch_interval(c, enc_w, nV * nH, (float)(wq - 0.5), d->init_layerwise, w_iv));
            if (sg.searches()) CHK(launch_cands(c, mult, w_iv, ncand, nV * nH, w_cands_ws));
        } else {
            CHK(launch_absmax(c, X, stw, 1, 1, M, K, 1, nA, M, crb_acts, d->twin_postgelu ? 1 : 0, enc_a));
            CHK(launch_interval(c, enc_a, nA, (float)(aq - 0.5), d->init_layerwise, a_iv));
            if (sg.searches()) CHK(launch_cands(c, mult, a_iv, ncand, nA, a_cands_ws));
        }
        return 0;
    }

    Operand x_operand(bool expanded, const float* scales, int sc_cs) const {
        Operand op{};
        op.present = true; op.expanded = expanded;
        op.pk = pack2d(X, M, K, K);
        op.pk.scales = scales; op.pk.sc_cs = sc_cs;
        op.pk.lo = -aq; op.pk.hi = aq - 1;
        if (nA > 1) { op.pk.blk_mode = 1; op.pk.blk_div = INT_MAX; op.pk.nblk_r = 1; op.pk.nblk_k = nA; op.pk.blk_div2 = crb_acts; }
        if (d->twin_postgelu) {
            if (i8) { op.pk.lo = 0; }
            else { op.pk.mode = PACK_TWIN_SIM; op.pk.lo = -aq; op.pk.neg_scale = a_neg; }
        }
        return op;
    }
    Operand xneg_operand() const {
        Operand op{};
        op.present = true; op.expanded = false;
        op.pk = pack2d(X, M, K, K);
        op.pk.scales = nullptr; op.pk.neg_scale = a_neg; op.pk.lo = -aq; op.pk.hi = 0;
        return op;
    }
    Operand w_operand(bool expanded, const float* scales, int sc_cs, bool by_vblock) const {
        Operand op{};
        op.present = true; op.expanded = expanded;
        if (by_vblock) {
            op.pk = pack2d(W, crb_rows, K, K);
            op.pk.s_z = (long)crb_rows * K;
            op.pk.blk_mode = 2; op.pk.blk_div = nV;
            if (nH > 1) return op;
        } else {
            op.pk = pack2d(W, N, K, K);
            op.pk.blk_mode = 1; op.pk.blk_div = crb_rows; op.pk.nblk_r = nV; op.pk.nblk_k = nH;
            op.pk.blk_div2 = nH > 1 ? crb_cols : 0;
        }
        op.pk.scales = scales; op.pk.sc_cs = sc_cs;
        op.pk.lo = -wq; op.pk.hi = wq - 1;
        return op;
    }

    Pass forward_pass() const {
        Pass fp{};
        fp.i8 = i8; fp.twin = twin; fp.epi = EPI_FWD; fp.wt_mode = 0; fp.eq_n = 1; fp.K = K;
        fp.Z = 1; fp.Mrows = M; fp.Ncols = N;
        fp.row = x_operand(false, a_iv, 0);
        if (twin) fp.row2 = xneg_operand();
        fp.col = w_operand(false, w_iv, 0, false);
        fp.use_s1 = i8; fp.s_cs = nV; fp.sb_mode = 1; fp.sb_div = crb_rows;
        fp.s1 = ScaleParams{a_iv, 0, 0, 0.f, w_iv, 0, 1, 0.f, 0, 0, nullptr};
        fp.s2 = ScaleParams{nullptr, 0, 0, a_neg, w_iv, 0, 1, 0.f, 0, 0, nullptr};
        fp.bias = bias; fp.bias_axis = 0; fp.bias_zs = 0;
        fp.O = fwd_out; fp.G = nullptr; fp.o_ms = N; fp.o_ns = 1; fp.o_inner = INT_MAX;
        fp.nj = 1; fp.store_out = fwd_out;
        return fp;
    }

    void selection(Pass& ps, int side, int round, int blk) const {
        const bool ws = side == 0;
        ps.nj = ws ? nV : 1; ps.cands = ws ? w_cands : a_cands; ps.cand_cs = ws ? nV * nH : nA; ps.cand_js = ws ? nH : 0; ps.cand_off = blk;
        ps.interval = ws ? w_iv : a_iv; ps.out_js = ws ? nH : 0; ps.out_off = blk;
        if (blk == tab_blk) { ps.scores_out = rounds.scores_of(round, side); ps.best_out = rounds.best_of(round, side); }
        ps.scores_out_ld = nV;
    }
    Pass search_pass(int side, int round, int blk, const float* cands, bool host_sync_ok) {
        const bool ws = side == 0;
        const int cs = ws ? nV * nH : nA;
        Pass ps{};
        ps.i8 = i8; ps.twin = twin; ps.epi = epi; ps.wt_mode = wt_mode; ps.eq_n = d->eq_n; ps.K = K;
        ps.cache = (rounds.keep_planes && (ws ? nH : nA) == 1) ? &plane[side] : nullptr;
        ps.ecache = rounds.keep_planes ? &ecache[side] : nullptr;
        selection(ps, side, round, blk);
        const bool dense = !cosm || cos6 || cos7;
        const Operand xo = ws ? x_operand(false, a_iv, 0) : x_operand(true, cands, cs);
        const Operand wo = ws ? w_operand(true, cands, cs, !dense) : w_operand(false, w_iv, 0, !dense);
        ps.s1 = ws ? ScaleParams{a_iv, 0, 0, 0.f, w_cands, nV, 1, 0.f, 0, 0, nullptr} : ScaleParams{a_cands, 1, 0, 0.f, w_iv, 0, 1, 0.f, 0, 0, nullptr};
        ps.use_s1 = i8; ps.s_cs = nV;
        ps.bias = bias; ps.O = O; ps.o_inner = INT_MAX;
        if (dense) {
            ps.Z = 1; ps.Mrows = M; ps.Ncols = N;
            ps.row = xo; ps.col = wo;
            if (twin) { ps.row2 = xneg_operand(); ps.twin_disjoint = ws; }
            ps.sb_mode = 1; ps.sb_div = crb_rows;
            ps.s2 = ScaleParams{nullptr, 0, 0, a_neg, ws ? w_cands : w_iv, ws ? nV : 0, 1, 0.f, 0, 0, nullptr};
            ps.bias_axis = 0; ps.bias_zs = 0;
            ps.G = G; ps.o_zs = 0; ps.o_bs = 0; ps.o_ms = N; ps.o_ns = 1;
// ... 24 lines not shown
        sgp.cands = (ws ? w_cands : a_cands) + blk; sgp.cand_cs = ws ? nV * nH : nA; sgp.cand_hs = ws ? nH : 0;
        Pass ps{};
        ps.seg = &sgp; ps.i8 = true; ps.epi = EPI_COS; ps.eq_n = d->eq_n; ps.K = K;
        ps.Z = nV; ps.Mrows = crb_rows; ps.Ncols = M;
        ps.bias = bias; ps.bias_axis = 1; ps.bias_zs = crb_rows;
        ps.O = Ot;
        ps.cos_ZB = 1; ps.cos_ZV = nV; ps.cos_j_mode = ws ? 1 : 0;
        ps.norm = 1.0 / (double)d->tokens;
        selection(ps, side, round, blk);
        return ps;
    }

    int mix_candidates(int side, int blk) {
        if (c.dry) return 0;
        const bool ws = side == 0;
        const int n = ws ? nV * nH : nA, rows = ws ? nV : 1;
        const float* cands = ws ? w_cands : a_cands;
        float* mix = ws ? w_mix : a_mix;
        ScaleParams mp{};
        mp.x = ws ? w_iv : a_iv; mp.x_cs = 0; mp.x_js = 1; mp.y = nullptr; mp.y_const = 1.0f; mp.C = ncand; mp.nblk = n; mp.S = mix;
        CHK(launch_scale(c, mp));
        for (int v = 0; v < rows; ++v)
            CHK(q_copy2d(c, mix + v * nH + blk, sizeof(float) * n, cands + v * nH + blk, sizeof(float) * n, sizeof(float), ncand));
        return 0;
    }

    int fold_negative_plane(Pass& ps) {
        Pass fp = ps;
        fp.twin = false; fp.epi = EPI_STORE; fp.wt_mode = 0; fp.eq_n = 1;
        fp.row = xneg_operand(); fp.row2 = Operand{};
        fp.s1 = ps.s2;
        fp.store_out = Ufold; fp.cache = nullptr;
        fp.scores_out = nullptr; fp.best_out = nullptr;
        CHK(run_pass(c, fp));
        ps.twin = false; ps.row2 = Operand{};
        ps.O = Ufold; ps.bias = nullptr;
        ps.ecache = nullptr;
        slice.o_src = nullptr;
        slice2.o_src = nullptr;
        return 0;
    }

    int search_side(int side, int round, MemoSide& memo, HostCopy* host) {
        const bool ws = side == 0;
        const int nblk = ws ? nH : nA;
        const DevVecs key = ws ? DevVecs(a_iv, nA) : DevVecs(w_iv, nV * nH), val = ws ? DevVecs(w_iv, nV * nH) : DevVecs(a_iv, nA);
        bool hit = false;
        CHK(memo.restore(c, key, &host[1 - side], val, &host[side], &hit));
        for (int blk = 0; blk < nblk && !hit && (sg.mask & (ws ? ST_S1 : ST_S2)); ++blk) {
            if (only_blk >= 0 && blk != only_blk) continue;
            if (segcos) { Pass ps = seg_cos_pass(side, round, blk); CHK(run_pass(c, ps)); continue; }
            const float* cands = ws ? w_cands : a_cands;
            if (general && nblk > 1) { CHK(mix_candidates(side, blk)); cands = ws ? w_mix : a_mix; }
            Pass ps = search_pass(side, round, blk, cands, memo.on);
            if (!ws && twin && wt_mode <= 1) CHK(fold_negative_plane(ps));
            CHK(run_pass_pruned(c, ps));
        }
        return hit ? 0 : memo.record(c, val, &host[side]);
    }
};

int linear_impl(const p4v_linear_desc* d, const float* W, const float* bias, const float* X, const float* O,
                const float* G, const float* mult, float* w_iv, float* a_iv, float* scores_out, int32_t* best_out,
                Ctx& c, float* fwd_out = nullptr, const Stage& sg = Stage{}) {
    LinearCall L(c, d, sg);
    CHK(L.build(W, bias, X, O, G, mult, w_iv, a_iv, scores_out, best_out, fwd_out));
    CHK(L.init_side(0));
    if (fwd_out || !sg.full()) {
        CHK(q_wait_inputs(c));
        CHK(L.init_side(1));
    }
    if (!fwd_out && !sg.searches()) return 0;
    if (fwd_out) { Pass fp = L.forward_pass(); return run_pass(c, fp); }
    const SearchRounds& R = L.rounds;
    MirrorScope mirrors(c, R.memo_on, w_iv, a_iv);
    MemoSide memo[2];
    memo[0].on = R.memo_on && L.nH == 1;
    memo[1].on = R.memo_on && L.nA == 1;
    HostCopy host[2];
    if (sg.full()) {
        if (R.keep_planes && L.nH == 1 && !L.cosm && (sg.mask & ST_S1)) {
            Pass pp = L.search_pass(0, 0, 0, L.w_cands, R.memo_on);
            pp.pack_only = true;
            CHK(run_pass(c, pp));
        }
        CHK(q_wait_inputs(c));
        CHK(L.init_side(1));
    }
    if (L.segcos) CHK(enqueue(c, KERN(NchwRowsParams, k_nchw_to_rows), dim3(cdiv(L.N, 32), cdiv(L.M, 32), 1), dim3(256), 0, NchwRowsParams{O, L.M, L.N, L.Ot}));
    for (int round = 0; round < R.n_rounds; ++round)
        for (int side = 0; side < 2; ++side) CHK(L.search_side(side, round, memo[side], host));
    return 0;
}

struct MatMulBlocks {
    int nVA = 1, nHA = 1, nVB = 1, nHB = 1, v = 0, h = 0;
    bool any() const { return nVA != 1 || nHA != 1 || nVB != 1 || nHB != 1; }
};
int matmul_blocks_impl(const p4v_matmul_desc* d, const MatMulBlocks& mb, const float* A, const float* B, const float* O, const float* G,
                       const float* mult, float* A_iv, float* B_iv, float* split, float* scores_out, int32_t* best_out, Ctx& c,
                       float* fwd_out, const Stage& sg);

struct MatMulCall {
    static constexpr int NSPLIT = 20;
    Ctx& c;
    const p4v_matmul_desc* d;
    const Stage& sg;
    int H = 0, Z = 0, M = 0, K = 0, N = 0;
    int Aq = 0, Bq = 0;
    int epi = 0, wt_mode = 0, ncand = 0;
    bool cosm = false;
    const float *A = nullptr, *B = nullptr, *O = nullptr, *G = nullptr, *mult = nullptr;
    float *A_iv = nullptr, *B_iv = nullptr, *split = nullptr;
    float* fwd_out = nullptr;
    unsigned *enc_A = nullptr, *enc_B = nullptr;
    float *A_cands_ws = nullptr, *B_cands_ws = nullptr;
    const float *A_cands = nullptr, *B_cands = nullptr;
    float* split_cands = nullptr;
    float* A_headwise = nullptr;
    SearchRounds rounds;
    PlaneCache plane_A, plane_B;
    SliceCache slice;

    MatMulCall(Ctx& c_, const p4v_matmul_desc* d_, const Stage& sg_) : c(c_), d(d_), sg(sg_) {}

    int build(const float* A_, const float* B_, const float* O_, const float* G_, const float* mult_, float* A_iv_, float* B_iv_,
              float* split_, float* scores_out, int32_t* best_out, float* fwd_out_) {
        A = A_; B = B_; O = O_; G = G_; mult = mult_; A_iv = A_iv_; B_iv = B_iv_; split = split_; fwd_out = fwd_out_;
        H = d->heads; Z = d->batch * d->heads; M = d->M; K = d->K; N = d->N;
        if (Z <= 0 || M <= 0 || K <= 0 || N <= 0 || d->eq_n <= 0) return fail(P4V_ERR_INVALID, "matmul: non-positive dimension");
        if (d->A_bit > 8 || d->B_bit > 8 || d->A_bit < 2 || d->B_bit < 2) return fail(P4V_ERR_UNSUPPORTED, "matmul: bit widths 2..8 supported");
        Aq = 1 << (d->A_bit - 1); Bq = 1 << (d->B_bit - 1);
        metric_epi(d->metric, &epi, &wt_mode);
        cosm = epi == EPI_COS;
        if (wt_mode == 1 && !G && !fwd_out && sg.searches()) return fail(P4V_ERR_INVALID, "matmul: hessian metric needs raw_grad");
        if (d->sos && !split) return fail(P4V_ERR_INVALID, "matmul: sos needs d_split");
        ncand = d->eq_n + 1;
        rounds = SearchRounds(sg, d->search_round, d->reserved, d->eq_n, H, c, scores_out, best_out);
        return 0;
    }
    int workspace() {
        enc_A = c.ws.get<unsigned>(H);
        enc_B = c.ws.get<unsigned>(H);
        A_cands_ws = c.ws.get<float>((size_t)ncand * H);
        B_cands_ws = c.ws.get<float>((size_t)ncand * H);
        A_cands = (sg.mask & ST_INIT) ? A_cands_ws : sg.cands1;
        B_cands = (sg.mask & ST_INIT) ? B_cands_ws : sg.cands2;
        split_cands = c.ws.get<float>(NSPLIT);
        A_headwise = c.ws.get<float>(H);
        if (!c.ws.ok()) return fail(P4V_ERR_WORKSPACE, "workspace too small");
        return 0;
    }
    int init() {
        if (fwd_out || !(sg.mask & ST_INIT)) return 0;
        const long sa[4] = {d->a_stride[0], d->a_stride[1], d->a_stride[2], d->a_stride[3]};
        const long sb[4] = {d->b_stride[0], d->b_stride[1], d->b_stride[2], d->b_stride[3]};
        float* a_dst = d->sos ? A_headwise : A_iv;
        CHK(launch_absmax(c, A, sa, d->batch, H, M, K, 1, 1, M, K, 0, enc_A));
        CHK(launch_interval(c, enc_A, H, (float)(Aq - 0.5), d->init_layerwise, a_dst));
        CHK(launch_absmax(c, B, sb, d->batch, H, K, N, 1, 1, K, N, 0, enc_B));
        CHK(launch_interval(c, enc_B, H, (float)(Bq - 0.5), d->init_layerwise, B_iv));
        if (sg.searches()) {
            if (!d->sos) CHK(launch_cands(c, mult, A_iv, ncand, H, A_cands_ws));
            CHK(launch_cands(c, mult, B_iv, ncand, H, B_cands_ws));
        }
        return 0;
// ... 844 lines not shown
    return conv_search("p4v_conv_search_w_layerwise", 0, ST_S1, desc, d_weight, d_bias, d_x, d_out, d_grad, d_w_cands,
                       d_w_interval, const_cast<float*>(d_a_interval), d_scores, d_best, d_workspace, workspace_bytes, stream);
}

int p4v_conv_search_a(const p4v_conv_desc* desc, const float* d_weight, const float* d_bias, const float* d_x,
                      const float* d_out, const float* d_grad, const float* d_a_cands, const float* d_w_interval,
                      float* d_a_interval, float* d_scores, int32_t* d_best, void* d_workspace, size_t workspace_bytes,
                      void* stream) {
    if (desc && desc->a_bit >= 32) return fail(P4V_ERR_INVALID, "p4v_conv_search_a: a_bit >= 32 leaves the input unquantised (conv.py:600)");
    return conv_search("p4v_conv_search_a", -1, ST_S2, desc, d_weight, d_bias, d_x, d_out, d_grad, d_a_cands,
                       const_cast<float*>(d_w_interval), d_a_interval, d_scores, d_best, d_workspace, workspace_bytes, stream);
}

int p4v_score_argmax_gather(const float* d_scores, int32_t eq_n, int32_t n_blocks, const float* d_cands, float* d_interval,
                            int32_t* d_best, void* stream) {
    if (!d_scores || !d_cands || !d_interval || eq_n <= 0 || n_blocks <= 0)
        return fail(P4V_ERR_INVALID, "p4v_score_argmax_gather: bad argument");
    Ctx c{(hipStream_t)stream, Arena(nullptr, 0), false};
    SelectParams sl{d_scores, eq_n, n_blocks, d_cands, n_blocks, 1, 0, d_interval, 1, 0, nullptr, 0.0f, nullptr, 0, d_best};
    return launch_select(c, sl);
}

int p4v_quantize_i8(const float* d_x, int64_t rows, int64_t cols, int64_t cols_padded, const float* d_scales,
                    int64_t rows_per_scale, int32_t lo, int32_t hi, int8_t* d_q, void* stream) {
    if (!d_x || !d_scales || !d_q || rows <= 0 || cols <= 0 || cols_padded % 64 || cols_padded < cols || rows_per_scale <= 0)
        return fail(P4V_ERR_INVALID, "quantize_i8: bad argument");
    Ctx c{(hipStream_t)stream, Arena(nullptr, 0), false};
    PackParams p = pack2d(d_x, rows, cols, cols);
    p.Rp = (int)rows; p.Kp = (int)cols_padded; p.dst = d_q; p.C = 1;
    p.scales = d_scales; p.sc_cs = 0; p.blk_mode = 1; p.blk_div = (int)rows_per_scale;
    p.nblk_r = cdiv(rows, rows_per_scale); p.nblk_k = 1; p.lo = lo; p.hi = hi;
    return launch_pack<int8_t>(c, p);
}

int p4v_fake_quant(const float* d_x, int64_t rows, int64_t cols, const float* d_scales, int64_t rows_per_scale,
                   int32_t lo, int32_t hi, float* d_y, void* stream) {
    if (!d_x || !d_scales || !d_y || rows <= 0 || cols <= 0 || rows_per_scale <= 0)
        return fail(P4V_ERR_INVALID, "fake_quant: bad argument");
    const long n = rows * cols;
    hipLaunchKernelGGL(k_fake_quant_rows, dim3((unsigned)std::min<long>(cdiv(n, 256), 65536)), dim3(256), 0,
                       (hipStream_t)stream, d_x, (long)rows, (long)cols, d_scales, (long)rows_per_scale, (float)lo, (float)hi, d_y);
    HIPCHK(hipGetLastError());
    return 0;
}

int p4v_multi_copy(const int64_t* d_table, int32_t n, int64_t index, int64_t max_bytes, void* stream) {
    if (!d_table || n <= 0 || index < 0 || max_bytes <= 0) return fail(P4V_ERR_INVALID, "p4v_multi_copy: bad argument");
    static_assert(sizeof(long) == sizeof(int64_t), "table entries are 64-bit");
    const unsigned gx = (unsigned)std::max<long>(1, std::min<long>(cdiv(max_bytes / 16, 256 * 8), 256));
    hipLaunchKernelGGL(k_multi_copy, dim3(gx, (unsigned)n), dim3(256), 0, (hipStream_t)stream, (const long*)d_table, (long)index);
    HIPCHK(hipGetLastError());
    return 0;
}

thread_local double g_evt_overhead_ms = 0.0;
int p4v_stats_enable(int enable) {
    g_stat_on = enable != 0;
    if (g_stat_on) {
        hipEvent_t a, b;
        HIPCHK(hipEventCreate(&a));
        HIPCHK(hipEventCreate(&b));
        double best = 1e9;
        for (int i = 0; i < 32; ++i) {
            HIPCHK(hipEventRecord(a, nullptr));
            HIPCHK(hipEventRecord(b, nullptr));
            HIPCHK(hipEventSynchronize(b));
            float ms = 0;
            HIPCHK(hipEventElapsedTime(&ms, a, b));
            best = std::min(best, (double)ms);
        }
        hipEventDestroy(a);
        hipEventDestroy(b);
        g_evt_overhead_ms = best < 1e8 ? best : 0.0;
    }
    return 0;
}

static int stats_drain() {
    for (auto& r : g_stat_recs) {
        HIPCHK(hipEventSynchronize(r.b));
        float ms = 0;
        HIPCHK(hipEventElapsedTime(&ms, r.a, r.b));
        ms = (float)std::max(0.0, (double)ms - g_evt_overhead_ms);
        if (r.kind == 0 || (r.kind >= 2 && r.kind <= 9) || (r.kind >= 12 && r.kind <= 15)) { g_stats.sweep_i8_ms += ms; g_stats.sweep_i8_launches++; g_stats.sweep_i8_macs += r.macs; g_stats.sweep_i8_alg_macs += r.alg; }
        if (r.kind == 2) { g_stats.sweep6_ms += ms; g_stats.sweep6_launches++; g_stats.sweep6_macs += r.macs; g_stats.sweep6_alg_macs += r.alg; }
        if (r.kind == 3 || r.kind == 4) { g_stats.sweep7_ms += ms; g_stats.sweep7_launches++; g_stats.sweep7_macs += r.macs; g_stats.sweep7_alg_macs += r.alg; }
        if (r.kind == 4) { g_stats.sweep7_twin_ms += ms; g_stats.sweep7_twin_launches++; }
        if (r.kind == 1 || r.kind == 11) { g_stats.sweep_f32_ms += ms; g_stats.sweep_f32_launches++; g_stats.sweep_f32_macs += r.macs; g_stats.sweep_f32_alg_macs += r.alg; }
        hipEventDestroy(r.a);
        hipEventDestroy(r.b);
        r.ms = ms;
        g_stat_done.push_back(r);
    }
    g_stat_recs.clear();
    return 0;
}

int p4v_stats_reset(void) {
    int r = stats_drain();
    g_stats = p4v_kernel_stats{};
    g_stat_done.clear();
    g_memo_hits = 0; g_memo_misses = 0;
    return r;
}

int p4v_stats_get(p4v_kernel_stats* out) {
    if (!out) return fail(P4V_ERR_INVALID, "stats_get: null");
    int r = stats_drain();
    g_stats.memo_hits = g_memo_hits; g_stats.memo_misses = g_memo_misses;
    g_stats.event_overhead_ms = g_evt_overhead_ms;
    *out = g_stats;
    return r;
}

int p4v_stats_launches(p4v_launch_record* out, int64_t capacity, int64_t* count) {
    int r = stats_drain();
    if (r) return r;
    if (count) *count = (int64_t)g_stat_done.size();
    if (out)
        for (int64_t i = 0; i < capacity && i < (int64_t)g_stat_done.size(); ++i) {
            const StatRec& s = g_stat_done[(size_t)i];
            out[i] = p4v_launch_record{s.kind, s.stage, s.gx, s.gz, (double)s.ms, 2.0 * s.macs, 2.0 * s.alg, s.bytes};
        }
    return 0;
}

int p4v_prune_counters(int64_t* out4, int reset) {
    if (out4) for (int i = 0; i < 4; ++i) out4[i] = (int64_t)g_prune_cnt[i].load(std::memory_order_relaxed);
    if (reset) for (int i = 0; i < 4; ++i) g_prune_cnt[i].store(0, std::memory_order_relaxed);
    return 0;
}

int p4v_debug_set_variant(int variant, int force_generic) {
    if (variant < 0 || variant >= (1 << 30)) return fail(P4V_ERR_INVALID, "p4v_debug_set_variant: bad variant word");
    if (variant & ~VARIANT_KEPT) return fail(P4V_ERR_INVALID, "p4v_debug_set_variant: bits 0x%x select removed paths", variant & ~VARIANT_KEPT);
    g_variant_word.store(variant | (force_generic ? (1 << 30) : 0), std::memory_order_relaxed);
    return 0;
}

int p4v_debug_set_tuning(int key, int value) {
    if (key < 0 || key >= 16) return fail(P4V_ERR_INVALID, "p4v_debug_set_tuning: unknown key %d", key);
    if (key == TUNE_B1_PATH && tune_b1_removed(value)) return fail(P4V_ERR_INVALID, "p4v_debug_set_tuning: 12 = %d selects a removed path", value);
    g_tune[key].store(value, std::memory_order_relaxed);
    return 0;
}

int p4v_debug_set_arena_gap(size_t bytes) {
    if (bytes % 256) return fail(P4V_ERR_INVALID, "p4v_debug_set_arena_gap: %zu is not a multiple of the arena's 256-byte alignment", bytes);
    g_arena_gap.store(bytes, std::memory_order_relaxed);
    return 0;
}

int p4v_debug_arena_ranges(uint64_t* out, int cap) {
    const int n = (int)g_arena_ranges.size();
    for (int i = 0; out && i < std::min(n, cap); ++i) { out[2 * i] = g_arena_ranges[i].first; out[2 * i + 1] = g_arena_ranges[i].second; }
    return n;
}

int p4v_debug_sos_sweep(const p4v_matmul_desc* desc, const float* d_A, const float* d_B, const float* d_out, const float* d_grad,
                        int n_cands, int c_lo, int c_hi, int known_cands, float* d_scores, void* d_workspace, size_t workspace_bytes,
                        void* stream) {
    if (!desc || !d_A || !d_B || !d_out || !d_scores || !d_workspace) return fail(P4V_ERR_INVALID, "p4v_debug_sos_sweep: null pointer");
    if (!desc->sos || n_cands < 1 || n_cands > 20 || !sos_split_ok(desc->M, desc->K, desc->N, false))
        return fail(P4V_ERR_INVALID, "p4v_debug_sos_sweep: a split-of-softmax matmul of the one-kernel split search, 1..20 candidates");
    const SosDebugSweep dbg{n_cands, c_lo, c_hi, known_cands, d_scores};
    float* d_split = nullptr;
    CHK(ws_aligned(d_workspace));
    HIPCHK(hipMalloc(&d_split, 2 * sizeof(float)));
    Ctx c{(hipStream_t)stream, Arena(d_workspace, workspace_bytes), false};
    g_sos_debug = &dbg;
    const int rc = matmul_impl(desc, d_A, d_B, d_out, d_grad, nullptr, d_split + 1, nullptr, d_split, nullptr, nullptr, c, nullptr,
                               Stage{ST_S1, nullptr, nullptr});
    g_sos_debug = nullptr;
    (void)hipFree(d_split);
    return rc;
}

int p4v_debug_bound_totals(float* out, int64_t capacity, int64_t* count) {
    if (!out && !count) { g_b1_keep = true; g_b1_totals.clear(); return 0; }
    g_b1_keep = false;
    if (count) *count = (int64_t)g_b1_totals.size();
    if (out) std::copy(g_b1_totals.begin(), g_b1_totals.begin() + std::min<int64_t>(capacity, (int64_t)g_b1_totals.size()), out);
    return 0;
}

int p4v_debug_topk_rows(const float* d_mass, int segs, int n, int k, int32_t* d_idx, void* stream) {
    if (!d_mass || !d_idx || segs <= 0 || n <= 0 || k <= 0 || k > n) return fail(P4V_ERR_INVALID, "p4v_debug_topk_rows: bad argument");
    hipLaunchKernelGGL(k_topk_rows, dim3(segs), dim3(1024), 0, (hipStream_t)stream, TopkParams{d_mass, n, k, d_idx});
    HIPCHK(hipGetLastError());
    return 0;
}

int p4v_debug_pack_dual(const float* d_x, long rows, long cols, long cols_padded, int sos, int lo, int hi, int qmax,
                        const float* d_scale, float const_scale, int8_t* d_q1, int8_t* d_q2, void* stream) {
    if (!d_x || !d_scale || !d_q1 || !d_q2 || rows <= 0 || cols <= 0 || cols_padded % 64 || cols_padded < cols ||
        lo > 0 || hi < 0 || lo < -128 || hi > 127 || qmax < 2 || qmax > 128 || (!sos && !(const_scale > 0.0f)))
        return fail(P4V_ERR_INVALID, "p4v_debug_pack_dual: bad argument");
    PackParams p1 = pack2d(d_x, rows, cols, cols);
    p1.Rp = (int)rows; p1.Kp = (int)cols_padded; p1.C = 1; p1.scales = d_scale; p1.qm1 = (float)(qmax - 1);
    PackParams p2 = p1;
    p1.dst = d_q1; p2.dst = d_q2;
    if (sos) {
        p1.mode = PACK_SOS_HI; p2.mode = PACK_SOS_LO;
    } else {
        p1.lo = 0; p1.hi = hi; p2.lo = lo; p2.hi = 0; p2.scales = nullptr; p2.neg_scale = const_scale;
    }
    if (!dual_pack_ok(p1, p2)) return fail(P4V_ERR_INVALID, "p4v_debug_pack_dual: not a dual pair");
    Ctx c{(hipStream_t)stream, Arena(nullptr, 0), false};
    const long total = rows * (cols_padded / 16);
    if (total >= (1L << 31)) return fail(P4V_ERR_UNSUPPORTED, "p4v_debug_pack_dual: plane too large");
    return enqueue(c, KERN(PackDualParams, k_pack_dual), dim3((unsigned)std::min<long>(cdiv(total, 256), 256L * 64)), dim3(256), 0,
                   PackDualParams{p1, p2});
}

int p4v_debug_pack_cands(const float* d_x, long rows, long cols, long rows_padded, long cols_padded, int layout, int lo, int hi,
                         const float* d_scales, int n_cands, const int* d_crange, const unsigned char* d_done, int live_max,
                         int general, int8_t* d_q, void* stream) {
    if (!d_x || !d_scales || !d_q || rows <= 0 || cols <= 0 || rows_padded < rows || cols_padded % 64 || cols_padded < cols ||
        layout < 0 || layout > 3 || (layout == 3 && rows_padded % 64) || lo > hi || lo < -128 || hi > 127 || n_cands <= 0 ||
        (d_done && !d_crange) || (live_max >= 0 && !d_crange))
        return fail(P4V_ERR_INVALID, "p4v_debug_pack_cands: bad argument");
    Ctx c{(hipStream_t)stream, Arena(nullptr, 0), false};
    cvt_bias(c);
    PackParams p = pack2d(d_x, rows, cols, cols);
    p.Rp = (int)rows_padded; p.Kp = (int)cols_padded; p.dst = d_q; p.C = n_cands; p.c_inner = layout;
    p.scales = d_scales; p.sc_cs = 1; p.lo = lo; p.hi = hi;
    p.crange = d_crange; p.c_base = 0; p.done = d_done;
    g_pack_general.store(general ? 1 : 0, std::memory_order_relaxed);
    const int r = launch_pack<int8_t>(c, p, live_max);
    g_pack_general.store(0, std::memory_order_relaxed);
    return r;
}

int p4v_debug_gather_im2col(int batch, int in_channels, int height, int width, int kernel_h, int kernel_w, int stride_h, int stride_w,
                            int pad_h, int pad_w, int dil_h, int dil_w, const float* d_x, const int32_t* d_idx, int k, float* d_dst,
                            void* stream) {
    if (!d_x || !d_idx || !d_dst || k <= 0 || batch <= 0 || in_channels <= 0 || height <= 0 || width <= 0 || kernel_h <= 0 ||
        kernel_w <= 0 || stride_h <= 0 || stride_w <= 0 || pad_h < 0 || pad_w < 0 || dil_h <= 0 || dil_w <= 0)
        return fail(P4V_ERR_INVALID, "p4v_debug_gather_im2col: bad argument");
    const int num_h = height + 2 * pad_h - dil_h * (kernel_h - 1) - 1, num_w = width + 2 * pad_w - dil_w * (kernel_w - 1) - 1;
    if (num_h < 0 || num_w < 0) return fail(P4V_ERR_INVALID, "p4v_debug_gather_im2col: bad geometry");
    const int fh = num_h / stride_h + 1, fw = num_w / stride_w + 1;
    PackParams p{};
    p.src = d_x; p.conv = 1; p.ic = in_channels; p.H = height; p.W = width; p.kh = kernel_h; p.kw = kernel_w;
    p.sh = stride_h; p.sw = stride_w; p.ph = pad_h; p.pw = pad_w; p.dh = dil_h; p.dw = dil_w;
    p.fw = fw; p.L = fh * fw;
    p.Z = 1; p.s_z = 0; p.R = batch * fh * fw; p.K = in_channels * kernel_h * kernel_w; p.nblk_r = 1; p.nblk_k = 1;
    p.mode = PACK_RAW;
    Ctx c{(hipStream_t)stream, Arena(nullptr, 0), false};
    const long total = (long)k * p.K;
    return enqueue(c, KERN(GatherIm2colParams, k_gather_im2col), dim3((unsigned)std::min<long>(cdiv(total, 256), 256L * 16)), dim3(256), 0,
                   GatherIm2colParams{p, d_idx, k, d_dst});
}

int p4v_debug_prep_epi6(const float* d_o, const float* d_wt, const float* d_bias, long o_ss, long o_ts, int sr, int tr,
                        int bias_on_t, int wt_mode, int transposed, float* d_e, void* stream) {
    if (!d_o || !d_bias || !d_e || (wt_mode == 1 && !d_wt) || sr <= 0 || tr <= 0 || wt_mode < 0 || wt_mode > 4)
        return fail(P4V_ERR_INVALID, "p4v_debug_prep_epi6: bad argument");
// ... 63 lines not shown
```

### ptq4vit_amd/csrc/p4v_kernels.h

```cpp
#pragma once
#include <hip/hip_runtime.h>
#include <stdint.h>
#include <type_traits>

namespace p4v {

typedef int v4i __attribute__((ext_vector_type(4)));
typedef int v16i __attribute__((ext_vector_type(16)));
typedef float v4f __attribute__((ext_vector_type(4)));
typedef float v16f __attribute__((ext_vector_type(16)));
typedef float v2f __attribute__((ext_vector_type(2)));

#ifndef P4V_GROUP_KERNARG
#define P4V_GROUP_KERNARG (4096 - 256)
#endif
template <typename P> struct GroupArgs {
    static constexpr int CAP_RAW = (P4V_GROUP_KERNARG - 16) / (int)(sizeof(P) + 16);
    static constexpr int CAP = CAP_RAW > 64 ? 64 : CAP_RAW;
    int n;
    unsigned off[CAP + 1];
    unsigned gx[CAP], gy[CAP], gz[CAP];
    P p[CAP];
};
#define P4V_BIDX uint3{blockIdx.x, blockIdx.y, blockIdx.z}
// ... 1772 lines not shown
__global__ __launch_bounds__(256, 2) void k_slice_b2(SliceB2Params p) { k_slice_b2_body<TWIN, KTM, NBW, EPI, SAT8>(p, P4V_BIDX, P4V_GDIM); }
template <bool TWIN, int KTM, int NBW, int EPI, bool SAT8>
__global__ __launch_bounds__(256, 2) void k_slice_b2_g(GroupArgs<SliceB2Params> a) { P4V_GROUP_ENTER(a); k_slice_b2_body<TWIN, KTM, NBW, EPI, SAT8>(a.p[m_], vb_, vg_); }

struct SliceAParams {
    const float* A;
    const int8_t* B;
    const float* ascale; int as_cs, as_div;
    int lo, hi;
    const float* S1; int s_cs, s_div;
    const float* O; const float* Wt; int wt_mode;
    int Z, M, K, N, C;
    float* part;
    float qbias;
};
template <int NBM, int EPI>
__device__ __forceinline__ void k_slice_a_body(const SliceAParams& p, const uint3 blockIdx, const uint3 gridDim) {
    typedef int v4i_ __attribute__((ext_vector_type(4)));
    const int tid = threadIdx.x, lane = tid & 63;
    const int wid = __builtin_amdgcn_readfirstlane(tid >> 6);
    const int l15 = lane & 15, l4 = lane >> 4;
    const int z = blockIdx.x;
    const int nb = (p.N + 15) / 16;
    const int per = (p.C + gridDim.y - 1) / gridDim.y;
    const int c_lo = blockIdx.y * per, c_hi = min(p.C, c_lo + per);
    float x[16];
#pragma unroll
    for (int e = 0; e < 16; ++e) {
        const int k = l4 * 16 + e;
        x[e] = (l15 < p.M && k < p.K) ? p.A[((long)z * 16 + l15) * p.K + k] : 0.0f;
    }
    v4i_ fb[NBM];
    float u[NBM][4], w[NBM][4];
    const int wm = p.wt_mode;
#pragma unroll
    for (int j = 0; j < NBM; ++j) {
        fb[j] = *reinterpret_cast<const v4i_*>(p.B + ((long)z * nb * 16 + min(j, nb - 1) * 16 + l15) * 64 + l4 * 16);
#pragma unroll
        for (int e = 0; e < 4; ++e) {
            const int n = j * 16 + l15, m = 4 * l4 + e;
            const bool ok = j < nb && n < p.N && m < p.M;
            const long idx = ((long)z * 16 + min(m, 15)) * p.N + min(n, p.N - 1);
            const float o = p.O[idx], gw = p.Wt[idx];
            float wv;
            if (wm == 1) wv = gw; else if (wm == 2) wv = o; else if (wm == 3) wv = fabsf(o); else wv = 1.0f;
            u[j][e] = ok ? o : 0.0f;
            w[j][e] = ok ? wv : 0.0f;
        }
    }
    const int saz = p.as_div > 0 ? z % p.as_div : 0, ssz = p.s_div > 0 ? z % p.s_div : 0;
    const float flo = (float)p.lo, fhi = (float)p.hi;
    const bool wide = !(fmaxf(-flo, fhi) < 129.0f);
    for (int c = c_lo + wid; c < c_hi; c += 4) {
        const float s = p.ascale[(long)c * p.as_cs + saz];
        const float rcp = 1.0f / s;
        const float s1 = p.S1 ? p.S1[(long)c * p.s_cs + ssz] : 1.0f;
        v4i fa;
        if (p.qbias != 0.0f) quant16_sat8(x, s, rcp, p.qbias, fa);
        else quant16_any(x, s, rcp, flo, fhi, wide, fa);
        float sum = 0.0f;
        const v4i_ zero4 = {0, 0, 0, 0};
#pragma unroll
        for (int j = 0; j < NBM; ++j) {
            if (j < nb) {
                const v4i_ acc = __builtin_amdgcn_mfma_i32_16x16x64_i8(fa, fb[j], zero4, 0, 0, 0);
#pragma unroll
                for (int e = 0; e < 4; ++e) {
                    const float d = u[j][e] - (float)acc[e] * s1;
                    const float ww = w[j][e];
                    if (EPI == EPI_SQ_W) { const float t2 = ww * d; sum = fmaf(t2, t2, sum); }
                    else if (EPI == EPI_ABS) sum = fmaf(ww, fabsf(d), sum);
                    else sum = fmaf(ww * d, d, sum);
                }
            }
        }
        sum = wave_sum_dpp(sum);
        if (lane == 63) p.part[(long)c * p.Z + z] = sum;
    }
}
template <int NBM, int EPI>
__global__ __launch_bounds__(256, 2) void k_slice_a(SliceAParams p) { k_slice_a_body<NBM, EPI>(p, P4V_BIDX, P4V_GDIM); }
template <int NBM, int EPI>
__global__ __launch_bounds__(256, 2) void k_slice_a_g(GroupArgs<SliceAParams> a) { P4V_GROUP_ENTER(a); k_slice_a_body<NBM, EPI>(a.p[m_], vb_, vg_); }

template <bool TWIN, int EPI>
__device__ __forceinline__ void k_sweep2g_body(const SweepParams& p, const uint3 blockIdx, const uint3 gridDim) {
    extern __shared__ __attribute__((aligned(16))) char smem[];
    constexpr int NPL = TWIN ? 4 : 3;
    constexpr int PLANE = SW2_NS * SW2_TILE;
    float* res = reinterpret_cast<float*>(smem + NPL * PLANE);

    const int tid = threadIdx.x, lane = tid & 63;
    const int wid = __builtin_amdgcn_readfirstlane(tid >> 6);
    const int wr = wid >> 2, wc = wid & 3;
    const int g = lane >> 5, l31 = lane & 31;

    const int nwg = p.mtiles * p.ntiles;
    const int t = xcd_remap(blockIdx.x, nwg);
    constexpr int GM = 4;
    const int per_group = GM * p.ntiles;
    const int first_m = (t / per_group) * GM;
    const int gsz = min(p.mtiles - first_m, GM);
    const int mt = first_m + (t % per_group) % gsz, nt = (t % per_group) / gsz;
    const int z = blockIdx.y;
    const int m0 = mt * SW_BM, n0 = nt * SW_BN;
    const int per = 2 * ((p.c1 - p.c0 + 2 * gridDim.z - 1) / (2 * gridDim.z));
    int c_lo_ = p.c0 + blockIdx.z * per, c_hi_ = min(p.c1, c_lo_ + per);
    clip_crange(p.crange, c_lo_, c_hi_, true);
    const int c_lo = c_lo_, c_hi = c_hi_;
    if (c_lo >= c_hi) return;
    const int ncand = c_hi - c_lo, npairs = (ncand + 1) >> 1;

    const int n = n0 + wc * 32 + l31;
    const bool ncol_ok = n < p.N;
    const float* biasz = p.bias ? p.bias + (long)z * p.bias_zs : nullptr;
    const float bias_n = (biasz && ncol_ok) ? biasz[n] : 0.0f;
    const int nc = min(n, p.N - 1);
    const int mlane = m0 + wr * 64 + 4 * g;
    const int m0w = m0 + wr * 64;
    const int gl_max = min(4, p.M - 1), gl = min(4 * g, p.M - 1);
    const unsigned lane_off0 = (unsigned)(nc * (int)p.o_ns);
    const unsigned lane_off = lane_off0 + (unsigned)(gl * (int)p.o_ms);
    const float* Ou = p.O + (long)z * p.o_zs;
    const float* Wu = p.Wt + (long)z * p.o_zs;
    const unsigned m_g = p.wt_mode == 1 ? 0xffffffffu : 0u;
    const unsigned m_o = p.wt_mode == 2 ? 0xffffffffu : p.wt_mode == 3 ? 0x7fffffffu : 0u;
    const unsigned m_1 = p.wt_mode == 0 ? 0x3f800000u : 0u;

    const int nw0 = n0 + wc * 32;
    const int sb = __builtin_amdgcn_readfirstlane(p.sb_mode == 1 ? min(nw0 / p.sb_div, p.s_cs - 1) : p.sb_mode == 2 ? z % p.sb_div : 0);
    float* s1tab = res + per * 8;
    float* s2tab = s1tab + per * 8;
    for (int i = lane; i < per; i += 64) {
        const int cc = min(c_lo + i, c_hi - 1);
        s1tab[i * 8 + wid] = p.S1 ? p.S1[cc * p.s_cs + sb] : 1.0f;
        if (TWIN) s2tab[i * 8 + wid] = p.S2 ? p.S2[cc * p.s_cs + sb] : 1.0f;
    }

    const int ld_row = wid * 16 + (lane >> 2);
    const int ld_chunk = (lane & 3) ^ ((ld_row >> 2) & 3);
    const unsigned voff = (unsigned)(ld_row * p.ldk + ld_chunk * 16);
    const char* curA = (const char*)p.A + (long)z * p.a_zs + (long)m0 * p.ldk;
    const char* curA2 = TWIN ? (const char*)p.A2 + (long)z * p.a2_zs + (long)m0 * p.ldk : nullptr;
    const char* curB0 = (const char*)p.B + (long)z * p.b_zs + (long)n0 * p.ldk + (long)c_lo * p.b_cs;
    long b1_off = (c_lo + 1 < c_hi) ? p.b_cs : 0;
    const int ktiles = p.ktiles;
    const long krow = (long)ktiles * SW_BKB;
    const int lds_wave = wid * 1024;
    const int total = npairs * ktiles;
    int ikt = 0, ipair = 0;
    auto issue = [&](int stage) __attribute__((always_inline)) {
        char* s = smem + stage * SW2_TILE + lds_wave;
        glds16(curA + voff, s);
        if (TWIN) glds16(curA2 + voff, s + PLANE);
        glds16(curB0 + voff, s + (NPL - 2) * PLANE);
        glds16(curB0 + b1_off + voff, s + (NPL - 1) * PLANE);
        curA += SW_BKB; curB0 += SW_BKB;
        if (TWIN) curA2 += SW_BKB;
        if (++ikt == ktiles) {
            ikt = 0; ++ipair;
            curA -= krow; if (TWIN) curA2 -= krow;
            curB0 += 2 * p.b_cs - krow;
            b1_off = (c_lo + 2 * ipair + 1 < c_hi) ? p.b_cs : 0;
        }
    };

// ... 2271 lines not shown
```

### ptq4vit_amd/engine.py

```python
import ctypes as C

import torch

from . import _lib

_workspace = {}
_mult_cache = {}


def _require_cuda(t, what):
    if not t.is_cuda:
        raise RuntimeError(f"ptq4vit_amd: {what} must live on the GPU (got {t.device}); the calibration path has no CPU fallback")


def device_of(*tensors):
    for t in tensors:
        if t is not None and t.is_cuda:
            return t.device
    if not torch.cuda.is_available():
        raise RuntimeError("ptq4vit_amd: no GPU visible -- the HIP calibration engine needs an MI355X (no CPU fallback)")
    return torch.device("cuda", torch.cuda.current_device())


def to_dev(t, dev):
# ... 644 lines not shown
        rc = _lib.load().p4v_debug_topk_rows(ptr(mass), segs, n, int(k), ptr(out), stream_ptr(mass.device))
    _lib.check(rc, "p4v_debug_topk_rows")
    return out


def debug_pack_dual(x2d, *, sos, scale, lo, hi, qmax, const_scale=0.0):
    x2d = x2d.contiguous().float()
    rows, cols = x2d.shape
    colsp = (cols + 63) // 64 * 64
    q1 = torch.empty(rows, colsp, dtype=torch.int8, device=x2d.device)
    q2 = torch.empty_like(q1)
    sc = torch.tensor([float(scale)], dtype=torch.float32, device=x2d.device)
    with torch.cuda.device(x2d.device):
        rc = _lib.load().p4v_debug_pack_dual(ptr(x2d), rows, cols, colsp, int(bool(sos)), int(lo), int(hi), int(qmax), ptr(sc),
                                             float(const_scale), ptr(q1), ptr(q2), stream_ptr(x2d.device))
    _lib.check(rc, "p4v_debug_pack_dual")
    return q1[:, :cols], q2[:, :cols], q1, q2


def debug_pack_cands(x2d, scales, *, layout, lo, hi, rows_padded=None, crange=None, done=None, live_max=-1, general=False,
                     out=None):
    x2d = x2d.contiguous().float()
    scales = scales.contiguous().float()
    rows, cols = x2d.shape
    n = scales.numel()
    colsp = (cols + 63) // 64 * 64
    rowsp = rows if rows_padded is None else int(rows_padded)
    size = rowsp * colsp * (1 if layout == 3 else (n + 1) // 2 * 2 if layout == 2 else n)
    if out is None:
        out = torch.zeros(size, dtype=torch.int8, device=x2d.device)
    assert out.dtype == torch.int8 and out.is_contiguous() and out.numel() >= size
    with torch.cuda.device(x2d.device):
        rc = _lib.load().p4v_debug_pack_cands(ptr(x2d), rows, cols, rowsp, colsp, int(layout), int(lo), int(hi), ptr(scales), n,
                                              ptr(crange) if crange is not None else None,
                                              ptr(done) if done is not None else None, int(live_max), int(bool(general)),
                                              ptr(out), stream_ptr(x2d.device))
    _lib.check(rc, "p4v_debug_pack_cands")
    return out


def debug_gather_im2col(x, idx, *, kernel_size, stride, padding, dilation):
    assert x.is_cuda and x.dtype == torch.float32 and x.dim() == 4 and idx.is_cuda and idx.dtype == torch.int32 and idx.dim() == 1
    x, idx = x.contiguous(), idx.contiguous()
    b, ic, H, W = x.shape
    (kh, kw), (sh, sw), (ph, pw), (dh, dw) = kernel_size, stride, padding, dilation
    fh, fw = (H + 2 * ph - dh * (kh - 1) - 1) // sh + 1, (W + 2 * pw - dw * (kw - 1) - 1) // sw + 1
    if fh > 0 and fw > 0:
        assert idx.numel() > 0 and int(idx.min()) >= 0 and int(idx.max()) < b * fh * fw, "row index outside the im2col matrix"
    out = torch.full((idx.numel(), ic * kh * kw), float("nan"), dtype=torch.float32, device=x.device)
    with torch.cuda.device(x.device):
        rc = _lib.load().p4v_debug_gather_im2col(b, ic, H, W, kh, kw, sh, sw, ph, pw, dh, dw, ptr(x), ptr(idx), idx.numel(), ptr(out),
                                                 stream_ptr(x.device))
    _lib.check(rc, "p4v_debug_gather_im2col")
    return out


def debug_prep_epi6(o, wt, bias, *, o_ss, o_ts, sr, tr, bias_on_t, wt_mode, transposed):
    n = -(-sr // 256) * -(-tr // 64) * 256 * 64 * 2
    e = torch.full((n,), float("nan"), dtype=torch.float32, device=o.device)
    with torch.cuda.device(o.device):
        rc = _lib.load().p4v_debug_prep_epi6(ptr(o), ptr(wt) if wt is not None else None, ptr(bias), int(o_ss), int(o_ts),
                                             int(sr), int(tr), int(bias_on_t), int(wt_mode), int(transposed), ptr(e),
                                             stream_ptr(o.device))
    _lib.check(rc, "p4v_debug_prep_epi6")
    return e

def debug_sos_sweep(*, A, B, out, grad, A_bit, metric, crange=None, known_cands=-1, n_cands=20):
    lib = _lib.load()
    dev = device_of(A, B)
    A, B = to_dev(A, dev), to_dev(B, dev)
    out = to_dev(out, dev).contiguous()
    grad = to_dev(grad, dev).contiguous() if grad is not None else None
    d = _matmul_desc(A, B, A_bit, 8, metric, 100, 1, True, 0, 0)[1]
    ws = workspace(dev, _need(lib.p4v_matmul_workspace_bytes, d, "p4v_matmul_workspace_bytes"))
    scores = torch.full((int(n_cands),), float("nan"), dtype=torch.float32, device=dev)
    lo, hi = (-1, -1) if crange is None else (int(crange[0]), int(crange[1]))
    with torch.cuda.device(dev):
        rc = lib.p4v_debug_sos_sweep(C.byref(d), ptr(A), ptr(B), ptr(out), ptr(grad), int(n_cands), lo, hi, int(known_cands),
                                     ptr(scores), ptr(ws), ws.numel(), stream_ptr(dev))
    _lib.check(rc, "p4v_debug_sos_sweep")
    return scores


def stats_reset():
    _lib.load().p4v_stats_reset()


def stats_get():
    s = _lib.KernelStats()
    _lib.check(_lib.load().p4v_stats_get(C.byref(s)), "p4v_stats_get")
    return {k: getattr(s, k) for k, _ in _lib.KernelStats._fields_}


def prune_counters(reset=False):
    out = (C.c_int64 * 4)()
    _lib.check(_lib.load().p4v_prune_counters(out, int(bool(reset))), "p4v_prune_counters")
    return dict(zip(("staged", "staged_no_survivors", "kept_full_sweep", "not_eligible"), (int(v) for v in out)))


def stats_launches():
    lib = _lib.load()
    n = C.c_int64(0)
    _lib.check(lib.p4v_stats_launches(None, 0, C.byref(n)), "p4v_stats_launches")
    buf = (_lib.LaunchRecord * max(1, n.value))()
    _lib.check(lib.p4v_stats_launches(buf, n.value, C.byref(n)), "p4v_stats_launches")
    return [{"kernel": _lib.LAUNCH_KINDS.get(r.kind, str(r.kind)), "stage": _lib.LAUNCH_STAGES.get(r.stage, str(r.stage)),
             "grid_x": r.grid_x, "grid_z": r.grid_z, "ms": r.ms, "ops": r.ops, "alg_ops": r.alg_ops, "alg_bytes": r.alg_bytes}
            for r in buf[:n.value]]
```

Before: 684.2.

## Add fused slice-W kernel that quantizes weights in registers during the pruned row-slice pass

Adds k_slice_w, a kernel for the stage-A pruning pass on linear layers. It keeps the float weight rows in registers, quantizes them per candidate scale on the fly, and runs int8 MFMA against a small row slice of packed activations held in LDS. This avoids materializing the large expanded per-candidate weight plane. When this path is expected, packing of that plane is deferred, saving the memory traffic and workspace. The cost is heavy register use (launch bounds of one block per CU), re-quantization work for every candidate, and a long chain of eligibility conditions.

```diff
diff --git a/include/ptq4vit_hip_debug.h b/include/ptq4vit_hip_debug.h
--- a/include/ptq4vit_hip_debug.h
+++ b/include/ptq4vit_hip_debug.h
@@ -16,6 +16,10 @@
 int p4v_debug_sos_sweep(const p4v_matmul_desc* desc, const float* d_A, const float* d_B, const float* d_out, const float* d_grad,
                         int n_cands, int c_lo, int c_hi, int known_cands, float* d_scores, void* d_workspace, size_t workspace_bytes,
                         void* stream);
+int p4v_debug_slice_w(const float* d_weight, const float* d_bias, const float* d_x, const float* d_out, const float* d_grad,
+                      const float* d_cands, const float* d_a_interval, int rows, int K, int N, int n_V, int n_cands, int w_bit, int a_bit,
+                      int metric, int sweep_only, float* d_scores, int* kernel_out, size_t* need_bytes, void* d_workspace,
+                      size_t workspace_bytes, void* stream);
 int p4v_debug_topk_rows(const float* d_mass, int segs, int n, int k, int32_t* d_idx, void* stream);
 int p4v_debug_pack_dual(const float* d_x, long rows, long cols, long cols_padded, int sos, int lo, int hi, int qmax,
                         const float* d_scale, float const_scale, int8_t* d_q1, int8_t* d_q2, void* stream);
diff --git a/ptq4vit_amd/_lib.py b/ptq4vit_amd/_lib.py
--- a/ptq4vit_amd/_lib.py
+++ b/ptq4vit_amd/_lib.py
@@ -54,7 +54,7 @@
 
 
 LAUNCH_KINDS = {0: "k_sweep<int8>", 1: "k_sweep<float>", 2: "k_sweep6", 3: "k_sweep7", 4: "k_sweep7 (twin)", 5: "k_sweep4/5", 6: "k_sweep9",
-                7: "k_sweep8", 8: "k_sweep2g", 9: "k_sweep2", 11: "k_sos_split", 12: "k_bound", 13: "k_slice_b", 14: "k_slice_a", 15: "k_sweep_seg"}
+                7: "k_sweep8", 8: "k_sweep2g", 9: "k_sweep2", 11: "k_sos_split", 12: "k_bound", 13: "k_slice_b", 14: "k_slice_a", 15: "k_sweep_seg", 16: "k_slice_w"}
 LAUNCH_STAGES = {0: "full", 1: "A", 2: "B1", 3: "B2", 4: "A2"}
 
 
@@ -99,7 +99,7 @@
     "p4v_quantize_i8", "p4v_pack_plane_i8", "p4v_fake_quant", "p4v_export_quantize", "p4v_multi_copy",
     "p4v_stats_enable", "p4v_stats_reset", "p4v_stats_get", "p4v_stats_launches", "p4v_prune_counters",
     "p4v_debug_set_variant", "p4v_debug_set_tuning", "p4v_debug_bound_totals", "p4v_debug_topk_rows", "p4v_debug_pack_dual", "p4v_debug_prep_epi6",
-    "p4v_debug_pack_cands", "p4v_debug_gather_im2col", "p4v_debug_sos_sweep",
+    "p4v_debug_pack_cands", "p4v_debug_gather_im2col", "p4v_debug_sos_sweep", "p4v_debug_slice_w",
     "p4v_debug_set_arena_gap", "p4v_debug_arena_ranges",
 ]
 
@@ -187,6 +187,9 @@
     lib.p4v_debug_gather_im2col.argtypes = [C.c_int] * 12 + [fp, ip, C.c_int, fp, vp]
     lib.p4v_debug_sos_sweep.restype = C.c_int
     lib.p4v_debug_sos_sweep.argtypes = [C.POINTER(MatMulDesc), fp, fp, fp, fp, C.c_int, C.c_int, C.c_int, C.c_int, fp, vp, C.c_size_t, vp]
+    if hasattr(lib, "p4v_debug_slice_w"):
+        lib.p4v_debug_slice_w.restype = C.c_int
+        lib.p4v_debug_slice_w.argtypes = [fp] * 7 + [C.c_int] * 9 + [fp, C.POINTER(C.c_int), C.POINTER(C.c_size_t), vp, C.c_size_t, vp]
     lib.p4v_debug_prep_epi6.restype = C.c_int
     lib.p4v_debug_prep_epi6.argtypes = [fp, fp, fp, C.c_long, C.c_long, C.c_int, C.c_int, C.c_int, C.c_int, C.c_int, fp, vp]
     lib.p4v_debug_set_variant.restype = C.c_int
diff --git a/ptq4vit_amd/csrc/p4v_api.hip b/ptq4vit_amd/csrc/p4v_api.hip
--- a/ptq4vit_amd/csrc/p4v_api.hip
+++ b/ptq4vit_amd/csrc/p4v_api.hip
@@ -110,9 +110,9 @@
 std::atomic<int> g_variant_word{0};
 #define g_variant (g_variant_word.load(std::memory_order_relaxed) & 0x3fffffff)
 #define g_force_v1 ((g_variant_word.load(std::memory_order_relaxed) >> 30) & 1)
-std::atomic<int> g_tune[16];
+std::atomic<int> g_tune[17];
 enum { TUNE_CG6 = 0, TUNE_CG2 = 1, TUNE_CG2G = 2, TUNE_CG7 = 3, TUNE_PRINT = 4, TUNE_ORDER7 = 5, TUNE_P6 = 6, TUNE_PLANE_GIB = 7, TUNE_EPI6W = 8,
-       TUNE_LOOSE_PCT = 9, TUNE_SLICE_DIV = 10, TUNE_SLICE_SMALL = 11, TUNE_B1_PATH = 12, TUNE_TIER2 = 13, TUNE_TIER2_DIV = 14, TUNE_LOOSE_ROWS = 15 };
+       TUNE_LOOSE_PCT = 9, TUNE_SLICE_DIV = 10, TUNE_SLICE_SMALL = 11, TUNE_B1_PATH = 12, TUNE_TIER2 = 13, TUNE_TIER2_DIV = 14, TUNE_LOOSE_ROWS = 15, TUNE_SLICE_W = 16 };
 inline bool tune_b1_removed(int v) { return v == 1 || v == 2 || v == 3 || v == 5 || v == 6 || v == 8 || v == 10 || v == 12; }
 inline int tune(int k) { return g_tune[k].load(std::memory_order_relaxed); }
 inline bool b1_previous() { return tune(TUNE_B1_PATH) == 4; }
@@ -230,7 +230,7 @@
     long n_ops = 0, n_launches = 0, n_rounds = 0;
     hipEvent_t inputs_ready = nullptr;
     bool waited = false;
-    int last_par[16] = {};
+    int last_par[24] = {};
     int issue_kernels(std::vector<const QOp*>& ops);
     int issue_round();
     int sync(int slot);
@@ -267,7 +267,7 @@
 int Group::issue_kernels(std::vector<const QOp*>& ops) {
     const KernelDesc* kd = ops[0]->kd;
     const int total = (int)ops.size();
-    if (ops[0]->heavy && ops[0]->si.kind >= 0 && ops[0]->si.kind < 16) last_par[ops[0]->si.kind] = total;
+    if (ops[0]->heavy && ops[0]->si.kind >= 0 && ops[0]->si.kind < 24) last_par[ops[0]->si.kind] = total;
     if (!kd->many || total == 1) {
         for (const QOp* op : ops) { CHK(enqueue_now(st, *op, op->timed && stat_recs, stat_recs)); ++n_launches; }
         return 0;
@@ -548,7 +548,7 @@
 
 inline int lockstep(const Ctx& c, int kind) {
     if (!c.grp) return 1;
-    const int seen = (kind >= 0 && kind < 16) ? c.grp->last_par[kind] : 0;
+    const int seen = (kind >= 0 && kind < 24) ? c.grp->last_par[kind] : 0;
     return std::max(1, seen > 0 ? seen : c.par);
 }
 inline int cu_slots(const Ctx& c, int slots, int kind) { return std::max(8, slots / lockstep(c, kind)); }
@@ -891,6 +891,7 @@
     PlaneCache* cache;
     EpiCache* ecache;
     bool pack_only;
+    bool pack_defer;
     const SegPlan* seg;
 };
 
@@ -1448,7 +1449,7 @@
     PassBufs b{};
     CHK(pass_workspace(c, ps, pl, b));
     if (ps.pack_only) {
-        if (b.pc && ps.row.expanded != ps.col.expanded && !ps.crange) CHK(pack_expanded(c, ps, pl, b, 0, ps.eq_n));
+        if (b.pc && ps.row.expanded != ps.col.expanded && !ps.crange && !ps.pack_defer) CHK(pack_expanded(c, ps, pl, b, 0, ps.eq_n));
         c.ws.off = mark;
         return 0;
     }
@@ -1694,6 +1695,76 @@
         P4V_EPI4(a.epi, CHK(enqueue(c, KERN_T(SliceAParams, k_slice_a, 13, E), grid, block, 0, kp, sp)); break)
     }
     FinishParams fp{part, (long)Z, 1L, 1, 1, Z, 1, a.eq_n, a.j_mode, std::max(1, a.j_div), a.nj, a.norm, SA, nullptr};
+    CHK(launch_finish(c, fp));
+    c.ws.off = mark;
+    return 0;
+}
+
+constexpr long SLICE_W_LDS_BYTES = 160L * 1024;
+constexpr long SLICE_W_MIN_PLANE_BYTES = 32L << 20;
+inline int slice_w_rows_max(int K) { return (int)std::min<long>(256, SLICE_W_LDS_BYTES / rup(K, 64) / 16 * 16); }
+bool slice_w_layer(const Pass& a) {
+    const PackParams& w = a.col.pk;
+    const PackParams& r = a.row.pk;
+    if (tune(TUNE_SLICE_W) == 1 || g_force_v1) return false;
+    if (!(a.i8 && a.Z == 1 && a.col.expanded && !a.row.expanded && !a.twin && !a.store_out && !a.seg && !a.cos6 && !a.cos7 &&
+          a.epi != EPI_COS && a.epi != EPI_STORE && a.epi != EPI_FWD && a.epi != EPI_COS_T && a.use_s1 && a.sb_mode == 1 &&
+          a.j_mode == 1 && a.j_div == a.sb_div && a.bias_axis == 0 && a.nj == a.s_cs && a.o_ms == a.Ncols && a.o_ns == 1 &&
+          !a.o_bs && !a.o_nbs && rup(a.K, 64) <= 768)) return false;
+    if (w.conv || w.mode != PACK_SYM || !w.scales || w.s_k != 1 || w.zdiv > 0 || w.blk_mode != 1 || w.blk_div2 || w.blk_div != a.sb_div ||
+        w.nblk_r != a.s_cs || w.lo < -128 || w.hi > 127 || (a.s_cs > 1 && a.sb_div % 16 != 0)) return false;
+    if (r.mode != PACK_SYM || !r.scales || r.lo < -128 || r.hi > 127) return false;
+    return tune(TUNE_SLICE_W) == 2 || (long)a.eq_n * a.Ncols * rup(a.K, 64) >= SLICE_W_MIN_PLANE_BYTES;
+}
+bool slice_w_ok(const Pass& a) {
+    return slice_w_layer(a) && !a.crange && a.scores_keep && a.no_select && !a.row.pk.conv && a.row.pk.s_k == 1 &&
+           a.Mrows <= slice_w_rows_max(a.K) && (rup(a.K, 64) <= 192 || a.Mrows <= 128);
+}
+int run_slice_w(Ctx& c, Pass& a, float* SA, bool plan_only = false) {
+    const int K64 = (int)rup(a.K, 64), N = a.Ncols, nsub = cdiv(N, 16);
+    const int KTM = K64 <= 192 ? 3 : K64 <= 384 ? 6 : 12, Kp = KTM * 64;
+    const int RBM = (KTM == 3 && (plan_only || a.Mrows > 128)) ? 16 : 8, Rp = RBM * 16;
+    const size_t mark = c.ws.off;
+    int8_t* A1 = c.ws.get<int8_t>((size_t)Rp * Kp);
+    float* part = c.ws.get<float>((size_t)a.eq_n * nsub);
+    float* S1 = a.S1_pre ? a.S1_pre : c.ws.get<float>((size_t)a.eq_n * a.s_cs);
+    if (!c.ws.ok()) return fail(P4V_ERR_WORKSPACE, "workspace too small: need >= %zu bytes", c.ws.off);
+    if (plan_only) { c.ws.off = mark; return 0; }
+    if (!a.s_ready) {
+        a.s1.S = S1; a.s1.C = a.eq_n; a.s1.nblk = a.s_cs;
+        CHK(launch_scale(c, a.s1));
+    }
+    {
+        PackParams pk = a.row.pk;
+        pk.Rp = Rp; pk.Kp = Kp; pk.dst = A1; pk.Z = 1; pk.C = 1; pk.c_inner = 0;
+        CHK(launch_pack<int8_t>(c, pk));
+    }
+    if (!c.dry) {
+        const PackParams& w = a.col.pk;
+        SliceWParams kp{};
+        kp.A = A1; kp.W = w.src; kp.w_n = w.s_r;
+        kp.wscale = w.scales; kp.ws_cs = w.sc_cs; kp.ws_div = std::max(1, w.blk_div); kp.ws_nblk = std::max(1, w.nblk_r); kp.lo = w.lo; kp.hi = w.hi;
+        kp.S1 = S1; kp.s_cs = a.s_cs; kp.s_div = std::max(1, a.sb_div);
+        kp.bias = a.bias; kp.O = a.O; kp.Wt = a.G ? a.G : a.O; kp.wt_mode = a.wt_mode;
+        kp.M = a.Mrows; kp.K = a.K; kp.Kp = Kp; kp.Rp = Rp; kp.N = N; kp.C = a.eq_n; kp.part = part;
+        kp.qbias = (w.lo == -128 && w.hi == 127 && tune(TUNE_B1_PATH) != 11) ? cvt_bias(c) : 0.0f;
+        const int fblocks = cdiv(N, 64), ktn = KTM, rbn = RBM;
+        int groups = choose_cgroups(fblocks, a.eq_n, 1, cu_slots(c, 256, 16), 1.5 + 0.25 * ktn, 0.013 * ktn * (4 + rbn), 50);
+        if (tune(TUNE_CG2) > 0) groups = std::max(1, std::min(a.eq_n, tune(TUNE_CG2)));
+        const dim3 grid(fblocks, groups), block(256);
+        const size_t lds = (size_t)Rp * Kp;
+        const StatInfo si{16, 16.0 * nsub * (double)Rp * Kp * a.eq_n, (double)a.Mrows * N * a.K * a.eq_n, g_stage, fblocks, groups,
+                          4.0 * ((double)a.Mrows * a.K + (double)N * a.K) + (a.G ? 8.0 : 4.0) * (double)a.Mrows * N};
+        const StatInfo* sp = &si;
+        int r_ = 0;
+#define P4V_LAUNCH_SW(KTM, RBM)                                                                                                       \
+        P4V_EPI4(a.epi, r_ = (kp.qbias != 0.0f) ? enqueue(c, KERN_T(SliceWParams, k_slice_w, KTM, RBM, E, true), grid, block, lds, kp, sp)   \
+                                                : enqueue(c, KERN_T(SliceWParams, k_slice_w, KTM, RBM, E, false), grid, block, lds, kp, sp); break)
+        if (KTM == 3 && RBM == 16) { P4V_LAUNCH_SW(3, 16) } else if (KTM == 3) { P4V_LAUNCH_SW(3, 8) } else if (KTM == 6) { P4V_LAUNCH_SW(6, 8) } else { P4V_LAUNCH_SW(12, 8) }
+#undef P4V_LAUNCH_SW
+        if (r_) return r_;
+    }
+    FinishParams fp{part, (long)nsub, 0L, nsub, 1, 1, nsub, a.eq_n, 1, a.nj > 1 ? std::max(1, a.j_div / 16) : nsub, a.nj, a.norm, SA, nullptr};
     CHK(launch_finish(c, fp));
     c.ws.off = mark;
     return 0;
@@ -1785,7 +1856,8 @@
     const bool virt = ps.nj > 1 && ps.cand_off == 0 && ps.cand_js * ps.nj == ps.cand_cs && ps.cand_cs <= 4096;
     PruneParams pp{SA, SB, ps.eq_n, ps.nj, prune_margin(), r1, r1, virt ? 1 : 0, best_idx, ps.cands, ps.cand_cs, ps.cand_js, ps.cand_off, vrow};
     g_stage = 1;
-    { const int r_ = slice_b_ok(a) ? run_slice_b(c, a, SA) : slice_a_ok(a) ? run_slice_a(c, a, SA) : run_pass(c, a); g_stage = 0; if (r_) return r_; }
+    if (c.dry && lin && slice_w_layer(a)) CHK(run_slice_w(c, a, SA, true));
+    { const int r_ = slice_b_ok(a) ? run_slice_b(c, a, SA) : slice_a_ok(a) ? run_slice_a(c, a, SA) : (!c.dry && slice_w_ok(a)) ? run_slice_w(c, a, SA) : run_pass(c, a); g_stage = 0; if (r_) return r_; }
     CHK(enqueue(c, KERN(PruneParams, k_prune_pick), dim3(1), dim3(256), 0, pp));
     Pass b1 = ps;
     b1.scores_keep = SB; b1.no_select = true;
@@ -2301,6 +2373,14 @@
         return 0;
     }
 
+    bool slice_w_expected(const Pass& ps) const {
+        if (!prune_ok(ps) || !ps.scache || ps.scache->loose || !slice_w_layer(ps)) return false;
+        const int k_cap = (int)std::min<long>(rup(std::max(1, M / (tune(TUNE_SLICE_DIV) > 0 ? tune(TUNE_SLICE_DIV) : 16)), 256), rup(M, 256));
+        if ((long)k_cap * 5 > (long)M * 2) return false;
+        const int k = (ps.host_sync_ok && k_cap >= 512) ? (tune(TUNE_SLICE_SMALL) > 0 ? std::min(tune(TUNE_SLICE_SMALL), k_cap)
+                                                                                          : (int)std::min<long>(std::max<long>(128, rup(M / 64, 64)), k_cap / 2)) : k_cap;
+        return k <= slice_w_rows_max(K) && (rup(K, 64) <= 192 || k <= 128);
+    }
     Operand x_operand(bool expanded, const float* scales, int sc_cs) const {
         Operand op{};
         op.present = true; op.expanded = expanded;
@@ -2491,6 +2571,7 @@
         if (R.keep_planes && L.nH == 1 && !L.cosm && (sg.mask & ST_S1)) {
             Pass pp = L.search_pass(0, 0, 0, L.w_cands, R.memo_on);
             pp.pack_only = true;
+            pp.pack_defer = !c.dry && L.slice_w_expected(pp);
             CHK(run_pass(c, pp));
         }
         CHK(q_wait_inputs(c));
@@ -3501,7 +3582,7 @@
         float ms = 0;
         HIPCHK(hipEventElapsedTime(&ms, r.a, r.b));
         ms = (float)std::max(0.0, (double)ms - g_evt_overhead_ms);
-        if (r.kind == 0 || (r.kind >= 2 && r.kind <= 9) || (r.kind >= 12 && r.kind <= 15)) { g_stats.sweep_i8_ms += ms; g_stats.sweep_i8_launches++; g_stats.sweep_i8_macs += r.macs; g_stats.sweep_i8_alg_macs += r.alg; }
+        if (r.kind == 0 || (r.kind >= 2 && r.kind <= 9) || (r.kind >= 12 && r.kind <= 16)) { g_stats.sweep_i8_ms += ms; g_stats.sweep_i8_launches++; g_stats.sweep_i8_macs += r.macs; g_stats.sweep_i8_alg_macs += r.alg; }
         if (r.kind == 2) { g_stats.sweep6_ms += ms; g_stats.sweep6_launches++; g_stats.sweep6_macs += r.macs; g_stats.sweep6_alg_macs += r.alg; }
         if (r.kind == 3 || r.kind == 4) { g_stats.sweep7_ms += ms; g_stats.sweep7_launches++; g_stats.sweep7_macs += r.macs; g_stats.sweep7_alg_macs += r.alg; }
         if (r.kind == 4) { g_stats.sweep7_twin_ms += ms; g_stats.sweep7_twin_launches++; }
@@ -3558,7 +3639,7 @@
 }
 
 int p4v_debug_set_tuning(int key, int value) {
-    if (key < 0 || key >= 16) return fail(P4V_ERR_INVALID, "p4v_debug_set_tuning: unknown key %d", key);
+    if (key < 0 || key >= 17) return fail(P4V_ERR_INVALID, "p4v_debug_set_tuning: unknown key %d", key);
     if (key == TUNE_B1_PATH && tune_b1_removed(value)) return fail(P4V_ERR_INVALID, "p4v_debug_set_tuning: 12 = %d selects a removed path", value);
     g_tune[key].store(value, std::memory_order_relaxed);
     return 0;
@@ -3593,6 +3674,46 @@
     g_sos_debug = nullptr;
     (void)hipFree(d_split);
     return rc;
+}
+
+int p4v_debug_slice_w(const float* d_weight, const float* d_bias, const float* d_x, const float* d_out, const float* d_grad,
+                      const float* d_cands, const float* d_a_interval, int rows, int K, int N, int n_V, int n_cands, int w_bit, int a_bit,
+                      int metric, int sweep_only, float* d_scores, int* kernel_out, size_t* need_bytes, void* d_workspace,
+                      size_t workspace_bytes, void* stream) {
+    if (rows <= 0 || K <= 0 || N <= 0 || n_V <= 0 || N % n_V || n_cands <= 0 || w_bit < 2 || w_bit > 8 || a_bit < 2 || a_bit > 8)
+        return fail(P4V_ERR_INVALID, "p4v_debug_slice_w: bad geometry");
+    const bool dry = d_workspace == nullptr;
+    if (!dry && (!d_weight || !d_x || !d_out || !d_cands || !d_a_interval || !d_scores)) return fail(P4V_ERR_INVALID, "p4v_debug_slice_w: null pointer");
+    if (!dry) CHK(ws_aligned(d_workspace));
+    Ctx c{(hipStream_t)stream, dry ? Arena(nullptr, 0) : Arena(d_workspace, workspace_bytes), dry};
+    cvt_bias(c);
+    int epi = 0, wt_mode = 0;
+    metric_epi(metric, &epi, &wt_mode);
+    if (epi == EPI_COS) return fail(P4V_ERR_INVALID, "p4v_debug_slice_w: a difference metric");
+    if (wt_mode == 1 && !d_grad && !dry) return fail(P4V_ERR_INVALID, "p4v_debug_slice_w: hessian needs d_grad");
+    const int wq = 1 << (w_bit - 1), aq = 1 << (a_bit - 1), crb = N / n_V;
+    Pass a{};
+    a.i8 = true; a.epi = epi; a.wt_mode = wt_mode; a.eq_n = n_cands; a.K = K; a.Z = 1; a.Mrows = rows; a.Ncols = N;
+    a.row.present = true; a.row.pk = pack2d(d_x, rows, K, K); a.row.pk.scales = d_a_interval; a.row.pk.lo = -aq; a.row.pk.hi = aq - 1;
+    a.col.present = true; a.col.expanded = true; a.col.pk = pack2d(d_weight, N, K, K);
+    a.col.pk.blk_mode = 1; a.col.pk.blk_div = crb; a.col.pk.nblk_r = n_V; a.col.pk.nblk_k = 1;
+    a.col.pk.scales = d_cands; a.col.pk.sc_cs = n_V; a.col.pk.lo = -wq; a.col.pk.hi = wq - 1;
+    a.s1 = ScaleParams{d_a_interval, 0, 0, 0.f, d_cands, n_V, 1, 0.f, 0, 0, nullptr};
+    a.use_s1 = true; a.s_cs = n_V; a.sb_mode = 1; a.sb_div = crb;
+    a.bias = d_bias; a.O = d_out; a.G = wt_mode == 1 ? d_grad : nullptr; a.o_inner = INT_MAX; a.o_ms = N; a.o_ns = 1;
+    a.j_mode = 1; a.j_div = crb; a.nj = n_V; a.norm = 1.0 / ((double)rows * crb);
+    a.scores_keep = d_scores; a.no_select = true;
+    const bool sw = !sweep_only && slice_w_ok(a);
+    if (kernel_out) *kernel_out = sw ? 1 : 0;
+    g_stage = 1;
+    int rc = 0;
+    if (dry) { if (slice_w_layer(a)) rc = run_slice_w(c, a, d_scores, true); if (!rc) rc = run_pass(c, a); }
+    else rc = sw ? run_slice_w(c, a, d_scores) : run_pass(c, a);
+    g_stage = 0;
+    if (need_bytes) *need_bytes = c.ws.peak + 4096;
+    if (rc || dry) return rc;
+    HIPCHK(hipStreamSynchronize((hipStream_t)stream));
+    return 0;
 }
 
 int p4v_debug_bound_totals(float* out, int64_t capacity, int64_t* count) {
diff --git a/ptq4vit_amd/csrc/p4v_kernels.h b/ptq4vit_amd/csrc/p4v_kernels.h
--- a/ptq4vit_amd/csrc/p4v_kernels.h
+++ b/ptq4vit_amd/csrc/p4v_kernels.h
@@ -1878,6 +1878,120 @@
 __global__ __launch_bounds__(256, 2) void k_slice_a(SliceAParams p) { k_slice_a_body<NBM, EPI>(p, P4V_BIDX, P4V_GDIM); }
 template <int NBM, int EPI>
 __global__ __launch_bounds__(256, 2) void k_slice_a_g(GroupArgs<SliceAParams> a) { P4V_GROUP_ENTER(a); k_slice_a_body<NBM, EPI>(a.p[m_], vb_, vg_); }
+
+struct SliceWParams {
+    const int8_t* A;
+    const float* W; long w_n;
+    const float* wscale; int ws_cs, ws_div, ws_nblk;
+    int lo, hi;
+    const float* S1; int s_cs, s_div;
+    const float* bias;
+    const float* O; const float* Wt; int wt_mode;
+    int M, K, Kp, Rp, N, C;
+    float* part;
+    float qbias;
+};
+template <int KTM, int RBM, int EPI, bool SAT8>
+__device__ __forceinline__ void k_slice_w_body(const SliceWParams& p, const uint3 blockIdx, const uint3 gridDim) {
+    extern __shared__ __attribute__((aligned(16))) unsigned char slw_lds[];
+    const int tid = threadIdx.x, lane = tid & 63;
+    const int wid = __builtin_amdgcn_readfirstlane(tid >> 6);
+    const int l15 = lane & 15, l4 = lane >> 4;
+    constexpr int ktn = KTM;
+    const int nsub = (p.N + 15) / 16;
+    const int per = (p.C + gridDim.y - 1) / gridDim.y;
+    const int c_lo = blockIdx.y * per, c_hi = min(p.C, c_lo + per);
+    {
+        const int kc = p.Kp / 16, chunks = p.Rp * kc;
+        for (int i = tid; i < chunks; i += 256) {
+            const int r = i / kc, q = i - r * kc;
+            const int dst = (((r >> 4) * ktn + (q >> 2)) * 64 + (q & 3) * 16 + (r & 15)) * 16;
+            *reinterpret_cast<v4i*>(slw_lds + dst) = *reinterpret_cast<const v4i*>(p.A + (long)i * 16);
+        }
+    }
+    const int j16 = blockIdx.x * 4 + wid;
+    const int n = j16 * 16 + l15, nc = min(n, p.N - 1);
+    float xw[KTM][16];
+    const float* wrow = p.W + (long)nc * p.w_n;
+    const bool vec = ((p.K | (int)p.w_n) & 3) == 0 && ((((unsigned long long)p.W) & 15) == 0);
+#pragma unroll
+    for (int kt = 0; kt < KTM; ++kt)
+#pragma unroll
+        for (int e4 = 0; e4 < 4; ++e4) {
+            const int k = kt * 64 + l4 * 16 + e4 * 4;
+            if (vec) {
+                const v4f v = *reinterpret_cast<const v4f*>(wrow + min(k, p.K - 4));
+                const bool ok = n < p.N && k < p.K;
+#pragma unroll
+                for (int e = 0; e < 4; ++e) xw[kt][e4 * 4 + e] = ok ? v[e] : 0.0f;
+            } else {
+#pragma unroll
+                for (int e = 0; e < 4; ++e) {
+                    const float v = wrow[min(k + e, p.K - 1)];
+                    xw[kt][e4 * 4 + e] = (n < p.N && k + e < p.K) ? v : 0.0f;
+                }
+            }
+        }
+    float u[RBM][4], w[RBM][4];
+    const int wm = p.wt_mode;
+    const float bn = p.bias ? p.bias[nc] : 0.0f;
+#pragma unroll
+    for (int rb = 0; rb < RBM; ++rb)
+#pragma unroll
+        for (int e = 0; e < 4; ++e) {
+            const int m = rb * 16 + 4 * l4 + e;
+            const bool ok = n < p.N && m < p.M;
+            const long idx = (long)min(m, p.M - 1) * p.N + nc;
+            const float o = p.O[idx], gw = p.Wt[idx];
+            float wv;
+            if (wm == 1) wv = gw; else if (wm == 2) wv = o; else if (wm == 3) wv = fabsf(o); else wv = 1.0f;
+            u[rb][e] = ok ? o - bn : 0.0f;
+            w[rb][e] = ok ? wv : 0.0f;
+        }
+    __syncthreads();
+    if (j16 >= nsub) return;
+    const int n0 = j16 * 16;
+    const int sbw = min(n0 / p.ws_div, p.ws_nblk - 1), sbs = min(n0 / p.s_div, p.s_cs - 1);
+    const float flo = (float)p.lo, fhi = (float)p.hi;
+    const bool wide = !(fmaxf(-flo, fhi) < 129.0f);
+    const unsigned char* frag = slw_lds + lane * 16;
+    for (int c = c_lo; c < c_hi; ++c) {
+        const float s = p.wscale[(long)c * p.ws_cs + sbw];
+        const float rcp = 1.0f / s;
+        const float s1 = p.S1[(long)c * p.s_cs + sbs];
+        v4i acc[RBM];
+#pragma unroll
+        for (int rb = 0; rb < RBM; ++rb) acc[rb] = v4i{0, 0, 0, 0};
+#pragma unroll
+        for (int kt = 0; kt < KTM; ++kt) {
+            v4i fa[RBM];
+#pragma unroll
+            for (int rb = 0; rb < RBM; ++rb) fa[rb] = *reinterpret_cast<const v4i*>(frag + (rb * ktn + kt) * 1024);
+            v4i fb;
+            if constexpr (SAT8) quant16_sat8(xw[kt], s, rcp, p.qbias, fb);
+            else quant16_any(xw[kt], s, rcp, flo, fhi, wide, fb);
+#pragma unroll
+            for (int rb = 0; rb < RBM; ++rb) acc[rb] = __builtin_amdgcn_mfma_i32_16x16x64_i8(fa[rb], fb, acc[rb], 0, 0, 0);
+        }
+        float sum = 0.0f;
+#pragma unroll
+        for (int rb = 0; rb < RBM; ++rb)
+#pragma unroll
+            for (int e = 0; e < 4; ++e) {
+                const float d = u[rb][e] - (float)acc[rb][e] * s1;
+                const float ww = w[rb][e];
+                if (EPI == EPI_SQ_W) { const float t2 = ww * d; sum = fmaf(t2, t2, sum); }
+                else if (EPI == EPI_ABS) sum = fmaf(ww, fabsf(d), sum);
+                else sum = fmaf(ww * d, d, sum);
+            }
+        sum = wave_sum_dpp(sum);
+        if (lane == 63) p.part[(long)c * nsub + j16] = sum;
+    }
+}
+template <int KTM, int RBM, int EPI, bool SAT8>
+__global__ __launch_bounds__(256, 1) void k_slice_w(SliceWParams p) { k_slice_w_body<KTM, RBM, EPI, SAT8>(p, P4V_BIDX, P4V_GDIM); }
+template <int KTM, int RBM, int EPI, bool SAT8>
+__global__ __launch_bounds__(256, 1) void k_slice_w_g(GroupArgs<SliceWParams> a) { P4V_GROUP_ENTER(a); k_slice_w_body<KTM, RBM, EPI, SAT8>(a.p[m_], vb_, vg_); }
 
 template <bool TWIN, int EPI>
 __device__ __forceinline__ void k_sweep2g_body(const SweepParams& p, const uint3 blockIdx, const uint3 gridDim) {
diff --git a/ptq4vit_amd/engine.py b/ptq4vit_amd/engine.py
--- a/ptq4vit_amd/engine.py
+++ b/ptq4vit_amd/engine.py
@@ -750,6 +750,27 @@
     return scores
 
 
+def debug_slice_w(*, weight, bias, x, out, grad, cands, a_interval, w_bit=8, a_bit=8, metric="hessian", sweep_only=False):
+    lib = _lib.load()
+    dev = device_of(weight, x)
+    f = lambda t: to_dev(t, dev).contiguous().float() if t is not None else None
+    weight, bias, x, out, grad, cands, a_interval = f(weight), f(bias), f(x), f(out), f(grad), f(cands), f(a_interval)
+    rows, K = x.shape
+    N = weight.shape[0]
+    n_cands, n_V = cands.shape
+    scores = torch.full((n_cands, n_V), float("nan"), dtype=torch.float32, device=dev)
+    kern, need = C.c_int(-1), C.c_size_t(0)
+    args = (ptr(weight), ptr(bias) if bias is not None else None, ptr(x), ptr(out), ptr(grad) if grad is not None else None,
+            ptr(cands), ptr(a_interval), int(rows), int(K), int(N), int(n_V), int(n_cands), int(w_bit), int(a_bit),
+            metric_id(metric), int(bool(sweep_only)), ptr(scores), C.byref(kern), C.byref(need))
+    _lib.check(lib.p4v_debug_slice_w(*args, None, 0, None), "p4v_debug_slice_w (sizing)")
+    ws = workspace(dev, need.value)
+    with torch.cuda.device(dev):
+        rc = lib.p4v_debug_slice_w(*args, ptr(ws), ws.numel(), stream_ptr(dev))
+    _lib.check(rc, "p4v_debug_slice_w")
+    return scores, ("k_slice_w" if kern.value == 1 else "sweep")
+
+
 def stats_reset():
     _lib.load().p4v_stats_reset()
 
```

New measurement: 690.7 (median of 3 runs). No clear change (+1.0%).
